# mzbac/mlx_sharding

Measured on AMD Instinct MI355X. Metric: output tokens/sec (decode), deepseek-v2-lite PP, higher is better.
Workload: dtype bf16; 1 GPU; model=deepseek-v2-lite, global_batch=64, seq_len=512, parallelism=pp1, micro_batches=1, weights=int4-w4a16

## Files before the change

### mlx_sharding_amd/models/deepseek_v2.py

```python

from __future__ import annotations

from typing import Dict, List, Optional, Tuple

import torch
import torch.nn as nn

from .. import ops
from ..config import ModelConfig, QuantConfig, ShardSpec
from ..ops.kvcache import KVCache
from .base import Linear, RMSNorm, StageModel, owned_layer_indices
from .llama import LlamaMLP, _Inner


class SwitchMLP(nn.Module):

    def __init__(self, n_experts: int, hidden: int, inter: int,
                 quant: Optional[QuantConfig] = None,
                 dtype: torch.dtype = torch.bfloat16):
        super().__init__()
        self.n_experts = n_experts
        self.quant = quant
        self.gate_proj = _StackedLinear(n_experts, hidden, inter, quant, dtype)
        self.up_proj = _StackedLinear(n_experts, hidden, inter, quant, dtype)
        self.down_proj = _StackedLinear(n_experts, inter, hidden, quant, dtype)

    def resident_dense(self):
        if self.quant is None:
            return None
        g, u, d = self.gate_proj, self.up_proj, self.down_proj
        return ops.expert_dequant_resident(
            (g.weight, g.scales, g.biases),
            (u.weight, u.scales, u.biases),
            (d.weight, d.scales, d.biases),
            self.quant.group_size, self.quant.bits)

    def forward_subs(self, x_flat: torch.Tensor, subs,
                     max_tok: int = 4) -> torch.Tensor:
        if self.quant is not None:
            import os
            if os.environ.get("MLXS_AMD_MOE_RESIDENT"):
                dense = self.resident_dense()
                if dense is not None:
                    return ops.grouped_expert_mlp_subs(
                        x_flat, dense[0], dense[1], dense[2], subs, max_tok)
            g, u, d = self.gate_proj, self.up_proj, self.down_proj
            return ops.grouped_expert_mlp_quant_subs(
                x_flat,
                (g.weight, g.scales, g.biases),
                (u.weight, u.scales, u.biases),
                (d.weight, d.scales, d.biases),
                subs, self.quant.group_size, self.quant.bits)
        return ops.grouped_expert_mlp_subs(
            x_flat, self.gate_proj.weight, self.up_proj.weight,
            self.down_proj.weight, subs, max_tok)

    def forward(self, x_flat: torch.Tensor, weights: torch.Tensor,
                indices: torch.Tensor) -> torch.Tensor:
        if self.quant is not None:
            g, u, d = self.gate_proj, self.up_proj, self.down_proj
            return ops.grouped_expert_mlp_quant(
                x_flat,
                (g.weight, g.scales, g.biases),
                (u.weight, u.scales, u.biases),
                (d.weight, d.scales, d.biases),
                weights, indices, self.quant.group_size, self.quant.bits)
        return ops.grouped_expert_mlp(
            x_flat, self.gate_proj.weight, self.up_proj.weight,
            self.down_proj.weight, weights, indices)


class _StackedLinear(nn.Module):

    def __init__(self, E: int, in_features: int, out_features: int,
                 quant: Optional[QuantConfig], dtype: torch.dtype):
        super().__init__()
        self.quantc = quant
        if quant is None:
            self.weight = nn.Parameter(
                torch.empty(E, out_features, in_features, dtype=dtype),
                requires_grad=False)
        else:
            per_word = 32 // quant.bits
            wdtype = torch.uint32 if hasattr(torch, "uint32") else torch.int32
            self.weight = nn.Parameter(
                torch.empty(E, out_features, in_features // per_word, dtype=wdtype),
                requires_grad=False)
            self.scales = nn.Parameter(
                torch.empty(E, out_features, in_features // quant.group_size, dtype=dtype),
                requires_grad=False)
            self.biases = nn.Parameter(
                torch.empty(E, out_features, in_features // quant.group_size, dtype=dtype),
                requires_grad=False)

    def dense(self) -> torch.Tensor:
        if self.quantc is None:
            return self.weight
        outs = [ops.dequantize(self.weight[e], self.scales[e], self.biases[e],
                               self.quantc.group_size, self.quantc.bits)
                for e in range(self.weight.shape[0])]
        return torch.stack(outs)


class MLAAttention(nn.Module):
    def __init__(self, cfg: ModelConfig, quant_for, prefix: str):
        super().__init__()
        H = cfg.hidden_size
        self.n_heads = cfg["num_attention_heads"]
        self.qk_nope = int(cfg.get("qk_nope_head_dim", 128))
        self.qk_rope = int(cfg.get("qk_rope_head_dim", 64))
        self.v_head_dim = int(cfg.get("v_head_dim", 128))
        self.kv_lora_rank = int(cfg.get("kv_lora_rank", 512))
        self.q_lora_rank = cfg.get("q_lora_rank")
        self.qk_head_dim = self.qk_nope + self.qk_rope
        q = lambda name: quant_for(f"{prefix}.{name}")
        eps = cfg.get("rms_norm_eps", 1e-6)
        if self.q_lora_rank:
            self.q_a_proj = Linear(H, self.q_lora_rank, q("q_a_proj"))
            self.q_a_layernorm = RMSNorm(self.q_lora_rank, eps)
            self.q_b_proj = Linear(self.q_lora_rank, self.n_heads * self.qk_head_dim,
                                   q("q_b_proj"))
        else:
            self.q_proj = Linear(H, self.n_heads * self.qk_head_dim, q("q_proj"))
        self._fused_qkv = None
        self.kv_a_proj_with_mqa = Linear(H, self.kv_lora_rank + self.qk_rope,
                                         q("kv_a_proj_with_mqa"))
        self.kv_a_layernorm = RMSNorm(self.kv_lora_rank, eps)
        self.kv_b_proj = Linear(self.kv_lora_rank,
                                self.n_heads * (self.qk_nope + self.v_head_dim),
                                q("kv_b_proj"))
        self.o_proj = Linear(self.n_heads * self.v_head_dim, H, q("o_proj"))

        rs = cfg.get("rope_scaling") or {}
        mscale_all = float(rs.get("mscale_all_dim", 0.0) or 0.0)
        factor = float(rs.get("factor", 1.0))
        scale = self.qk_head_dim ** -0.5
        if mscale_all and factor > 1.0:
            scale = scale * ops.yarn_mscale(factor, mscale_all) ** 2
        self.scale = scale
        self._w_uk = None
        self._w_uv = None

    def absorbed_supported(self) -> bool:
        ext = ops.hip_ext()
        if ext is None:
            return False
        dk = self.kv_lora_rank + self.qk_rope
        return (dk % 8 == 0 and self.kv_lora_rank % 8 == 0
                and ext.attn_decode_shape_ok(self.n_heads, self.kv_lora_rank))

    def _ensure_absorb(self, device, dtype):
        if self._w_uk is not None:
            return
        w = self.kv_b_proj.weight
        if self.kv_b_proj.quant is not None:
            qc = self.kv_b_proj.quant
            w = ops.dequantize(w, self.kv_b_proj.scales, self.kv_b_proj.biases,
                               qc.group_size, qc.bits)
        w = w.to(device=device, dtype=dtype)
        w = w.view(self.n_heads, self.qk_nope + self.v_head_dim,
                   self.kv_lora_rank)
        self._w_uk = w[:, : self.qk_nope, :].contiguous()
        self._w_uv = w[:, self.qk_nope:, :].transpose(1, 2).contiguous()

    def forward(self, x, cos, sin, cache: Optional[KVCache]):
        if cache is not None and cache.n_kv_heads == 1 and self.n_heads > 1:
            return self._forward_absorbed(x, cos, sin, cache)
        return self._forward_naive(x, cos, sin, cache)

    def _forward_absorbed(self, x, cos, sin, cache: KVCache):
        B, T, _ = x.shape
        nh, rank, rope = self.n_heads, self.kv_lora_rank, self.qk_rope
        ckv = None
        if self._fused_qkv is not None:
            qh, ckv = self._fused_qkv(x)
        elif self.q_lora_rank:
            qh = self.q_b_proj(self.q_a_layernorm(self.q_a_proj(x)))
        else:
            qh = self.q_proj(x)
        qh = qh.view(B, T, nh, self.qk_head_dim)
        q_nope = qh[..., : self.qk_nope]
        q_pe = ops.apply_rope(qh[..., self.qk_nope:], cos, sin,
                              interleaved=True)

        if ckv is None:
            ckv = self.kv_a_proj_with_mqa(x)
        c_kv, k_pe = ckv.split([rank, rope], dim=-1)
        c_kv = self.kv_a_layernorm(c_kv)
        k_pe = ops.apply_rope(k_pe.view(B, T, 1, rope), cos, sin,
                              interleaved=True).view(B, T, rope)

        gp = cache.graph_pos
        offset = 0 if gp is not None else cache.offset
        if ops.use_native(x):
            k_all, _ = cache.append_mla(c_kv.reshape(B, T, 1, rank), k_pe)
        else:
            row = torch.cat([c_kv, k_pe], dim=-1).unsqueeze(1)
            k_all, _ = cache.update(row, row[..., :0])

        if T == 1:
            self._ensure_absorb(x.device, x.dtype)
            qn = q_nope.permute(2, 0, 1, 3).reshape(nh, B * T, self.qk_nope)
            q_abs = torch.bmm(qn, self._w_uk)
            qf = torch.cat([q_abs.view(nh, B, T, rank).permute(1, 0, 2, 3),
                            q_pe.transpose(1, 2)], dim=-1)
            o = ops.attention(qf, k_all, k_all[..., :rank], self.scale,
                              causal_offset=offset, pos_dev=gp)
            ov = torch.bmm(o.permute(1, 0, 2, 3).reshape(nh, B * T, rank),
                           self._w_uv)
            out = ov.view(nh, B, T, self.v_head_dim).permute(1, 2, 0, 3)
            return self.o_proj(out.reshape(B, T, -1))

        S = k_all.shape[2] if gp is not None else cache.offset
        ckv_all = k_all[:, 0, :S, :rank]
        kpe_all = k_all[:, 0, :S, rank:]
        kvh = self.kv_b_proj(ckv_all).view(B, S, nh,
                                           self.qk_nope + self.v_head_dim)
        ext = ops.hip_ext() if ops.use_native(x) else None
        if ext is not None:
            k = kvh.new_empty(B, nh, S, self.qk_head_dim)
            v = kvh.new_empty(B, nh, S, self.v_head_dim)
            ext.mla_append_kv(kvh, kpe_all, k, v, pos0=0)
        else:
            k = torch.cat([kvh[..., : self.qk_nope],
                           kpe_all.reshape(B, S, 1, rope)
                           .expand(B, S, nh, rope)],
                          dim=-1).transpose(1, 2).contiguous()
            v = kvh[..., self.qk_nope:].transpose(1, 2).contiguous()
        qf = torch.cat([q_nope, q_pe], dim=-1).transpose(1, 2)
        out = ops.attention(qf, k, v, self.scale, causal_offset=offset)
        return self.o_proj(out.transpose(1, 2).reshape(B, T, -1))

    def _forward_naive(self, x, cos, sin, cache: Optional[KVCache]):
        B, T, _ = x.shape
        ckv = None
        if self._fused_qkv is not None:
            qh, ckv = self._fused_qkv(x)
        elif self.q_lora_rank:
            qh = self.q_b_proj(self.q_a_layernorm(self.q_a_proj(x)))
        else:
            qh = self.q_proj(x)
        qh = qh.view(B, T, self.n_heads, self.qk_head_dim)
        q_nope = qh[..., : self.qk_nope]
        q_pe = qh[..., self.qk_nope:]

        if ckv is None:
            ckv = self.kv_a_proj_with_mqa(x)
        c_kv, k_pe = ckv.split([self.kv_lora_rank, self.qk_rope], dim=-1)
        c_kv = self.kv_a_layernorm(c_kv)
        kvh = self.kv_b_proj(c_kv).view(B, T, self.n_heads, self.qk_nope + self.v_head_dim)

        q_pe = ops.apply_rope(q_pe, cos, sin, interleaved=True)
        k_pe = ops.apply_rope(k_pe.view(B, T, 1, self.qk_rope), cos, sin,
                              interleaved=True)
        qf = torch.cat([q_nope, q_pe], dim=-1).transpose(1, 2)

        offset = 0
        gp = None
        if cache is not None and ops.use_native(x):
            gp = cache.graph_pos
            if gp is None:
                offset = cache.offset
            k, v = cache.append_mla(kvh, k_pe.reshape(B, T, self.qk_rope))
            if gp is None:
                pass
        else:
            k_nope = kvh[..., : self.qk_nope]
            v = kvh[..., self.qk_nope:].transpose(1, 2)
            k = torch.cat([k_nope,
                           k_pe.expand(B, T, self.n_heads, self.qk_rope)],
                          dim=-1).transpose(1, 2)
            if cache is not None:
                gp = cache.graph_pos
                if gp is None:
                    offset = cache.offset
                k, v = cache.update(k, v)
        out = ops.attention(qf, k, v, self.scale, causal_offset=offset,
                            pos_dev=gp)
        return self.o_proj(out.transpose(1, 2).reshape(B, T, -1))


class DeepseekV2MoE(nn.Module):
    def __init__(self, cfg: ModelConfig, quant_for, prefix: str):
        super().__init__()
        H = cfg.hidden_size
        I_moe = int(cfg.get("moe_intermediate_size", 1408))
        self.n_experts = int(cfg.get("n_routed_experts", 64))
        self.top_k = int(cfg.get("num_experts_per_tok", 6))
        self.n_group = int(cfg.get("n_group", 1) or 1)
        self.topk_group = int(cfg.get("topk_group", 1) or 1)
        self.topk_method = cfg.get("topk_method", "greedy")
        self.routed_scaling_factor = float(cfg.get("routed_scaling_factor", 1.0))
        self.norm_topk_prob = bool(cfg.get("norm_topk_prob", False))
        self.gate = Linear(H, self.n_experts, None, dtype=torch.bfloat16)
        squant = quant_for(f"{prefix}.switch_mlp.gate_proj")
        self.switch_mlp = SwitchMLP(self.n_experts, H, I_moe, squant)
        n_shared = int(cfg.get("n_shared_experts", 0) or 0)
        if n_shared:
            shared_cfg = ModelConfig(cfg.model_type, dict(cfg.raw))
            shared_cfg.raw["intermediate_size"] = I_moe * n_shared
            self.shared_experts = LlamaMLP(shared_cfg, quant_for,
                                           f"{prefix}.shared_experts")
        else:
            self.shared_experts = None

    def _gate_groups(self) -> Tuple[int, int]:
        if self.topk_method == "group_limited_greedy":
            return self.n_group, self.topk_group
        return 1, 1

    def _fused_gate_ok(self, n_tokens: int) -> bool:
        E, K = self.n_experts, self.top_k
        n_group, topk_group = self._gate_groups()
        return (n_tokens <= 128 and 1 <= E <= 256 and 1 <= K <= 8
                and 1 <= n_group <= 32 and E % n_group == 0
                and 1 <= topk_group <= n_group
                and topk_group * (E // n_group) >= K)

    def forward(self, x):
        B, T, H = x.shape
        flat = x.reshape(-1, H)
        if (ops.use_native(flat)
                and self._fused_gate_ok(flat.shape[0])):
            logits = self.gate(flat.to(self.gate.weight.dtype))
            mt = 16
            n_group, topk_group = self._gate_groups()
            subs = ops.moe_gate_subranges(logits, self.top_k,
                                          self.routed_scaling_factor,
                                          self.norm_topk_prob, max_tok=mt,
                                          n_group=n_group,
                                          topk_group=topk_group)
            y = self.switch_mlp.forward_subs(flat, subs, mt)
        else:
            logits = self.gate(flat.to(self.gate.weight.dtype)).float()
            n_group = self.n_group if self.topk_method == "group_limited_greedy" else 1
            w, idx = ops.moe_gate(logits, self.top_k, n_group, self.topk_group,
                                  self.routed_scaling_factor, self.norm_topk_prob)
            w = w.to(x.dtype)
            y = self.switch_mlp(flat, w, idx)
        if self.shared_experts is not None:
            y = y + self.shared_experts(flat)
        return y.reshape(B, T, H)


class DeepseekV2DecoderLayer(nn.Module):
    def __init__(self, cfg: ModelConfig, quant_for, prefix: str, layer_idx: int):
        super().__init__()
        eps = cfg.get("rms_norm_eps", 1e-6)
        self.self_attn = MLAAttention(cfg, quant_for, f"{prefix}.self_attn")
        first_dense = int(cfg.get("first_k_dense_replace", 0))
        freq = int(cfg.get("moe_layer_freq", 1))
        is_moe = (cfg.get("n_routed_experts") is not None
                  and layer_idx >= first_dense and layer_idx % freq == 0)
        if is_moe:
            self.mlp = DeepseekV2MoE(cfg, quant_for, f"{prefix}.mlp")
        else:
            self.mlp = LlamaMLP(cfg, quant_for, f"{prefix}.mlp")
        self.input_layernorm = RMSNorm(cfg.hidden_size, eps)
        self.post_attention_layernorm = RMSNorm(cfg.hidden_size, eps)

    def forward(self, x, cos, sin, cache):
        attn = self.self_attn(self.input_layernorm(x), cos, sin, cache)
        pn = self.post_attention_layernorm
        y, h = ops.rms_norm_residual(attn, x, pn.weight, pn.eps,
                                     pn.weight_offset)
        return h + self.mlp(y)


class DeepseekV2StageModel(StageModel):
    model_type = "deepseek_v2"

    def __init__(self, config: ModelConfig, shard: ShardSpec, quant_for=None):
        super().__init__(config, shard)
        quant_for = quant_for or (lambda prefix: None)
        H = config.hidden_size
        self.model = _Inner()
        if shard.is_first:
            self.model.embed_tokens = nn.Embedding(config.vocab_size, H,
                                                   dtype=torch.bfloat16)
        layers = nn.ModuleDict()
        for i in owned_layer_indices(shard):
            layers[str(i)] = DeepseekV2DecoderLayer(config, quant_for,
                                                    f"model.layers.{i}", i)
        self.model.layers = layers
        if shard.is_last:
            self.model.norm = RMSNorm(H, config.get("rms_norm_eps", 1e-6))
            self.lm_head = Linear(H, config.vocab_size, quant_for("lm_head"))
        inv = ops.rope_freqs(int(config.get("qk_rope_head_dim", 64)),
                             float(config.get("rope_theta", 10000.0)),
                             config.get("rope_scaling"))
        rs = config.get("rope_scaling") or {}
        factor = float(rs.get("factor", 1.0))
        mscale = float(rs.get("mscale", 1.0) or 1.0)
        mscale_all = float(rs.get("mscale_all_dim", 0.0) or 0.0)
        if rs:
            num = ops.yarn_mscale(factor, mscale)
            den = ops.yarn_mscale(factor, mscale_all) if mscale_all else 1.0
            self.rope_attn_scale = num / den
        else:
            self.rope_attn_scale = 1.0
        self.register_buffer("rope_inv_freq", inv, persistent=False)

    @classmethod
    def sanitize(cls, weights: Dict[str, torch.Tensor], shard: ShardSpec) -> Dict[str, torch.Tensor]:
        out = dict(weights)
        expert_groups: Dict[str, Dict[int, str]] = {}
        for k in list(out.keys()):
            parts = k.split(".")
            if "experts" in parts and "shared_experts" not in k:
                ei = parts.index("experts")
                e = int(parts[ei + 1])
                stacked_key = ".".join(parts[:ei]) + ".switch_mlp." + ".".join(parts[ei + 2:])
                expert_groups.setdefault(stacked_key, {})[e] = k
        for stacked_key, members in expert_groups.items():
            n = max(members) + 1
            out[stacked_key] = torch.stack([out.pop(members[e]) for e in range(n)])
        return StageModel.sanitize.__func__(cls, out, shard)

    def cache_specs(self) -> List[Tuple[int, int, int]]:
        cfg = self.config
        if self._use_absorbed():
            rank = int(cfg.get("kv_lora_rank", 512))
            rope = int(cfg.get("qk_rope_head_dim", 64))
            return [(1, rank + rope, 0) for _ in range(self.shard.n_layers)]
        qk = int(cfg.get("qk_nope_head_dim", 128)) + int(cfg.get("qk_rope_head_dim", 64))
        vd = int(cfg.get("v_head_dim", 128))
        nh = cfg["num_attention_heads"]
        return [(nh, qk, vd) for _ in range(self.shard.n_layers)]

    def _use_absorbed(self) -> bool:
        try:
            p = next(self.parameters())
        except StopIteration:
            return False
        if not p.is_cuda:
            return False
        for layer in self.model.layers.values():
            return layer.self_attn.absorbed_supported()
        return False

    def forward(self, x: torch.Tensor, cache: Optional[List[KVCache]] = None) -> torch.Tensor:
        h = self.model.embed_tokens(x) if self.shard.is_first else x
        T = h.shape[1]
        cos, sin, _ = self.rope_for(cache[0] if cache else None, T, h.device)
        for j, i in enumerate(owned_layer_indices(self.shard)):
            c = cache[j] if cache is not None else None
            h = self.model.layers[str(i)](h, cos, sin, c)
        if self.shard.is_last:
            h = self.model.norm(h)
            h = self.lm_head(h)
        return h
```

### mlx_sharding_amd/ops/__init__.py

```python

from __future__ import annotations

import os
from typing import Optional

import torch

from . import reference as ref

_EXT = None
_EXT_ERR: Optional[str] = None
_TRIED = False


def _load_ext():
    global _EXT, _EXT_ERR, _TRIED
    if _TRIED:
        return _EXT
    _TRIED = True
    try:
        from mlx_sharding_amd import _hip_ops
        _EXT = _hip_ops
    except Exception as e:
        _EXT = None
        _EXT_ERR = repr(e)
    return _EXT


def hip_ext():
    return _load_ext()


def _force_torch() -> bool:
    return os.environ.get("MLXS_AMD_FORCE_TORCH", "0") == "1"


def _require_ext(op_name: str):
    ext = _load_ext()
    if ext is None:
        raise RuntimeError(
            f"mlx_sharding_amd: op '{op_name}' called on a GPU tensor but the "
            f"HIP extension mlx_sharding_amd._hip_ops is not importable "
            f"({_EXT_ERR}). Build it with `python setup.py build_ext --inplace` "
            f"(or __graft_entry__.build()). Refusing to fall back to eager torch "
            f"on GPU; set MLXS_AMD_FORCE_TORCH=1 only for debugging."
        )
    return ext


def _use_hip(t: torch.Tensor) -> bool:
    return t.is_cuda and not _force_torch()


def use_native(t: torch.Tensor) -> bool:
    return t.is_cuda and not _force_torch() and _load_ext() is not None



def rms_norm(x, weight, eps: float = 1e-5, weight_offset: float = 0.0):
    if _use_hip(x):
        return _require_ext("rms_norm").rms_norm(x, weight, eps, weight_offset)
    return ref.rms_norm(x, weight, eps, weight_offset)


def rms_norm_residual(x, residual, weight, eps: float = 1e-5, weight_offset: float = 0.0):
    if _use_hip(x):
        y, h = _require_ext("rms_norm_residual").rms_norm_residual(
            x, residual, weight, eps, weight_offset)
        return y, h
    h = x + residual
    return ref.rms_norm(h, weight, eps, weight_offset), h


def apply_rope(x, cos, sin, interleaved: bool = False):
    if _use_hip(x):
        return _require_ext("apply_rope").apply_rope(
            x, cos.contiguous(), sin.contiguous(), interleaved)
    return ref.apply_rope(x, cos, sin, interleaved)


def attention(q, k, v, scale: float, causal_offset: int = 0,
              softcap: float = 0.0, sliding_window: int = 0, pos_dev=None):
    if _use_hip(q):
        ext = _require_ext("attention")
        cache_layout = k.stride(3) == 1 and k.stride(2) == k.shape[3]
        if q.shape[2] == 1 and cache_layout:
            return ext.attn_decode(q, k, v, scale, softcap, sliding_window,
                                   pos_dev)
        if (cache_layout
                and ext.attn_prefill_shape_ok(q.shape[3], v.shape[3])):
            return ext.attn_prefill(q, k, v, scale, softcap, sliding_window,
                                    causal_offset)
        return _prefill_attention_gpu(q, k, v, scale, causal_offset,
                                      softcap, sliding_window)
    if pos_dev is not None:
        if pos_dev.numel() > 1:
            outs = []
            for b, p in enumerate(pos_dev.tolist()):
                outs.append(ref.attention(
                    q[b:b + 1], k[b:b + 1, :, :p + 1], v[b:b + 1, :, :p + 1],
                    scale, causal_offset=p, softcap=softcap,
                    sliding_window=sliding_window))
            return torch.cat(outs, dim=0)
        S = int(pos_dev.item()) + 1
        return ref.attention(q, k[:, :, :S], v[:, :, :S], scale,
                             causal_offset=S - 1, softcap=softcap,
                             sliding_window=sliding_window)
    return ref.attention(q, k, v, scale, causal_offset, softcap, sliding_window)


def _prefill_attention_gpu(q, k, v, scale, causal_offset, softcap, sliding_window):
    B, Hq, Tq, Dk = q.shape
    Hkv, S = k.shape[1], k.shape[2]
    G = Hq // Hkv
    qg = q.view(B, Hkv, G, Tq, Dk)
    scores = torch.matmul(qg, k.unsqueeze(2).transpose(-1, -2)).float() * scale
    if softcap and softcap > 0:
        scores = torch.tanh(scores / softcap) * softcap
    qpos = torch.arange(Tq, device=q.device)[:, None] + causal_offset
    kpos = torch.arange(S, device=q.device)[None, :]
    mask = kpos > qpos
    if sliding_window and sliding_window > 0:
        mask = mask | (kpos <= qpos - sliding_window)
    scores = scores.masked_fill(mask, float("-inf"))
    probs = torch.softmax(scores, dim=-1).to(q.dtype)
    out = torch.matmul(probs, v.unsqueeze(2))
    return out.reshape(B, Hq, Tq, v.shape[3])


def swiglu(gate, up):
    if _use_hip(gate):
        return _require_ext("swiglu").glu(gate, up, False)
    return ref.swiglu(gate, up)


def geglu(gate, up):
    if _use_hip(gate):
        return _require_ext("geglu").glu(gate, up, True)
    return ref.geglu(gate, up)


def softcap(x, cap: float):
    if _use_hip(x):
        return _require_ext("softcap").softcap(x, cap)
    return ref.softcap(x, cap)


_GEMV_MAX_M = 64
_LONG_K = 16384


_DQ_CACHE_BYTES = 0


def _dq_cache_cap() -> Optional[float]:
    if os.environ.get("MLXS_AMD_NO_DQ_CACHE"):
        return None
    return float(os.environ.get("MLXS_AMD_DQ_CACHE_GB", "96")) * (1 << 30)


def _dq_cache_ok(nbytes: int) -> bool:
    global _DQ_CACHE_BYTES
    cap = _dq_cache_cap()
    if cap is None or _DQ_CACHE_BYTES + nbytes > cap:
        return False
    _DQ_CACHE_BYTES += nbytes
    return True


def _small_m_route(M: int, O: int, K: int, x_dtype, w_dtype,
                   w_contiguous: bool, on_gpu: bool):
    if not (on_gpu and x_dtype == torch.bfloat16
            and w_dtype == torch.bfloat16 and w_contiguous
            and 0 < M <= _GEMV_MAX_M):
        return None
    if os.environ.get("MLXS_AMD_DENSE_GEMV") and K % 32 == 0:
        return "gemv", None
    if os.environ.get("MLXS_AMD_GEMM64") and K >= _LONG_K and K % 8 == 0:
        return "gemm64", None
    if (not os.environ.get("MLXS_AMD_NO_KSEG")
            and K >= _LONG_K and O >= 8192 and K % 256 == 0):
        return "kseg", max(1, min(16, 512 // max(1, O // 64)))
    return None


def _small_m_linear(x, weight, bias, name: str, ksegs):
    ext = _require_ext("linear")
    x2 = x.reshape(-1, x.shape[-1])
    if name == "gemv":
        y = ext.dense_gemv(x2, weight)
    elif name == "gemm64":
        y = ext.dense_gemm64(x2, weight)
    else:
        y = ext.gemm_m64_kseg(x2, weight, ksegs)
    if bias is not None:
        y = y + bias
    return y.reshape(*x.shape[:-1], y.shape[-1])


def linear(x, weight, bias=None):
    K = weight.shape[-1]
    if K >= _LONG_K or os.environ.get("MLXS_AMD_DENSE_GEMV"):
        route = _small_m_route(x.numel() // max(1, x.shape[-1]),
                               weight.shape[0], K, x.dtype, weight.dtype,
                               weight.is_contiguous(), _use_hip(x))
        if route is not None:
            return _small_m_linear(x, weight, bias, *route)
    return torch.nn.functional.linear(x, weight, bias)


def quantized_linear(x, w_q, scales, biases, group_size: int, bits: int):
    if _use_hip(x):
        ext = _require_ext("quantized_linear")
        lead = x.shape[:-1]
        H = x.shape[-1]
        x2 = x.reshape(-1, H)
        M = x2.shape[0]
        w = getattr(w_q, "_mlxs_dqw", None)
        O = w_q.shape[0]
        if w is None and _dq_cache_ok(O * H * 2):
            w = ext.dequant(w_q, scales, biases, H, group_size, bits)
            w_q._mlxs_dqw = w
        if w is not None:
            y = linear(x2, w)
        elif (M <= _GEMV_MAX_M and group_size in (32, 64, 128)
              and not os.environ.get("MLXS_AMD_NO_W4F16")):
            y = ext.w4f16_gemv(_to_f16_cached(x).reshape(-1, H),
                               repack_w4(w_q, bits),
                               scales, biases, group_size, bits)
        elif M <= _GEMV_MAX_M:
            y = ext.w4a16_gemv(x2, w_q, scales, biases, group_size, bits)
        else:
            w = ext.dequant(w_q, scales, biases, H, group_size, bits)
            y = torch.nn.functional.linear(x2, w)
        return y.reshape(*lead, y.shape[-1])
    return ref.quantized_linear(x, w_q, scales, biases, group_size, bits)


def moe_gate(router_logits, top_k: int, n_group: int = 1, topk_group: int = 1,
             routed_scaling_factor: float = 1.0, norm_topk_prob: bool = False):
    return ref.moe_gate(router_logits, top_k, n_group, topk_group,
                        routed_scaling_factor, norm_topk_prob)


_MOE_GEMM_MIN_N = 256


def make_expert_subranges(indices: torch.Tensor, weights: torch.Tensor,
                          n_experts: int, max_tok: int = 4):
    N, K = indices.shape
    P = N * K
    dev = indices.device
    flat_e = indices.reshape(-1).long()
    order = torch.argsort(flat_e, stable=True)
    tok = torch.arange(N, device=dev, dtype=torch.int64).repeat_interleave(K)
    sorted_tok = tok[order].to(torch.int32)
    sorted_wt = weights.reshape(-1).float()[order].contiguous()
    counts = torch.bincount(flat_e, minlength=n_experts)
    start = torch.cumsum(counts, 0) - counts
    nsub = (counts + max_tok - 1) // max_tok
    sub_start = torch.cumsum(nsub, 0) - nsub
    s_upper = n_experts + P // max_tok
    marker = torch.full((s_upper + 1,), -1, dtype=torch.int64, device=dev)
    eidx_all = torch.arange(n_experts, device=dev)
    src = torch.where(nsub > 0, eidx_all, torch.full_like(eidx_all, -1))
    marker.scatter_reduce_(0, sub_start, src, reduce="amax",
                           include_self=True)
    sub_expert = torch.cummax(marker[:s_upper], 0).values.clamp(min=0)
    sub_idx = torch.arange(s_upper, device=dev) - sub_start[sub_expert]
    sub_off = (start[sub_expert] + max_tok * sub_idx).to(torch.int32)
    sub_cnt = (counts[sub_expert] - max_tok * sub_idx) \
        .clamp(0, max_tok).to(torch.int32)
    return (sub_expert.to(torch.int32).contiguous(), sub_off.contiguous(),
            sub_cnt.contiguous(), sorted_tok.contiguous(), sorted_wt, order)


def _cached_t(w: torch.Tensor) -> torch.Tensor:
    if w.requires_grad or not w.is_leaf:
        return w.transpose(1, 2).contiguous()
    t = getattr(w, "_mlxs_t", None)
    if t is None:
        t = w.transpose(1, 2).contiguous()
        w._mlxs_t = t
    return t


def _cached_gu_t(gate_w: torch.Tensor, up_w: torch.Tensor) -> torch.Tensor:
    t = getattr(gate_w, "_mlxs_gut", None)
    if t is not None:
        return t
    E, I, H = gate_w.shape
    t = torch.empty(E, H, 2 * I, dtype=gate_w.dtype, device=gate_w.device)
    t[..., :I] = gate_w.transpose(1, 2)
    t[..., I:] = up_w.transpose(1, 2)
    if not gate_w.requires_grad and gate_w.is_leaf:
        gate_w._mlxs_gut = t
    return t


def _moe_prefill_gemm(x, gate_w, up_w, down_w, weights, indices,
                      dequant_all=None):
    N, K = indices.shape
    H = x.shape[-1]
    dev = x.device
    flat_e = indices.reshape(-1).long()
    order = torch.argsort(flat_e, stable=True)
    sorted_e = flat_e[order]
    tok = torch.arange(N, device=dev).repeat_interleave(K)[order]
    wts = weights.reshape(-1).float()[order]
    if dequant_all is not None:
        gate_w, up_w, down_w = dequant_all()
    E = gate_w.shape[0]
    counts = torch.zeros(E, dtype=torch.long, device=dev)
    counts.scatter_add_(0, sorted_e, torch.ones_like(sorted_e))
    start = torch.cumsum(counts, 0) - counts
    cap = (int(counts.max()) + 127) // 128 * 128
    P = N * K
    slot = torch.arange(P, device=dev) - start[sorted_e]
    dst = sorted_e * cap + slot
    xp = x.new_zeros(E * cap, H)
    ext = hip_ext() if x.is_cuda else None
    if ext is not None and H % 4 == 0:
        ext.moe_scatter_rows(x, xp, tok.to(torch.int32),
                             dst.to(torch.int32))
    else:
        xp[dst] = x[tok]
    xp = xp.view(E, cap, H)
    I = gate_w.shape[1]
    gu = torch.bmm(xp, _cached_gu_t(gate_w, up_w))
    hh = swiglu(gu[..., :I], gu[..., I:])
    d = torch.bmm(hh, _cached_t(down_w)).reshape(E * cap, H)
    if ext is not None and H % 4 == 0:
        inv = torch.empty_like(order)
        inv[order] = torch.arange(P, device=dev)
        pair_pos = dst[inv].view(N, K).to(torch.int32)
        pair_wts = weights.reshape(N, K).float()
        return ext.moe_gather_reduce(d, pair_pos, pair_wts, N)
    y = d[dst].float() * wts[:, None]
    out = torch.zeros(N, H, device=dev, dtype=torch.float32)
    out.index_add_(0, tok, y)
    return out.to(x.dtype)


def moe_gate_subranges(router_logits_bf16, top_k: int,
                       routed_scaling_factor: float = 1.0,
                       norm_topk_prob: bool = False, max_tok: int = 4,
                       n_group: int = 1, topk_group: int = 1):
    ext = _require_ext("moe_gate_subranges")
    N, E = router_logits_bf16.shape
    s_upper = E + (N * top_k) // max_tok
    return tuple(ext.moe_gate_subranges(router_logits_bf16, top_k, s_upper,
                                        max_tok, routed_scaling_factor,
                                        norm_topk_prob, n_group, topk_group))


def grouped_expert_mlp_subs(x, gate_w, up_w, down_w, subs, max_tok: int = 4):
    ext = _require_ext("grouped_expert_mlp")
    sub_e, sub_off, sub_cnt, sorted_tok, sorted_wt = subs
    P = sorted_tok.shape[0]
    h = ext.moe_gateup_grouped(x, gate_w, up_w, sub_e, sub_off, sub_cnt,
                               sorted_tok, P, max_tok)
    out = ext.moe_down_grouped(h, down_w, sub_e, sub_off, sub_cnt,
                               sorted_tok, sorted_wt, x.shape[0], max_tok)
    return out.to(x.dtype)


def _to_f16_cached(x: torch.Tensor) -> torch.Tensor:
    c = getattr(x, "_mlxs_f16", None)
    if c is not None:
        return c
    c = x.to(torch.float16)
    try:
        x._mlxs_f16 = c
    except Exception:
        pass
    return c


def repack_w4(wq: torch.Tensor, bits: int) -> torch.Tensor:
    cached = getattr(wq, "_mlxs_rp", None)
    if cached is not None:
        return cached
    w = wq.view(torch.int32).to(torch.int64) & 0xFFFFFFFF
    if bits == 4:
        even = ((w & 0xF) | (((w >> 8) & 0xF) << 4)
                | (((w >> 16) & 0xF) << 8) | (((w >> 24) & 0xF) << 12))
        odd = (((w >> 4) & 0xF) | (((w >> 12) & 0xF) << 4)
               | (((w >> 20) & 0xF) << 8) | (((w >> 28) & 0xF) << 12))
        rp = even | (odd << 16)
    elif bits == 8:
        rp = ((w & 0xFF) | (((w >> 16) & 0xFF) << 8)
              | (((w >> 8) & 0xFF) << 16) | (((w >> 24) & 0xFF) << 24))
    else:
        raise ValueError(f"unsupported bits {bits}")
    rp = torch.where(rp >= 2 ** 31, rp - 2 ** 32, rp).to(torch.int32)
    rp = rp.view(wq.dtype).contiguous()
    if not wq.requires_grad and wq.is_leaf:
        wq._mlxs_rp = rp
    return rp


def grouped_expert_mlp_quant_subs(x, gate, up, down, subs,
                                  group_size: int, bits: int):
    ext = _require_ext("grouped_expert_mlp_quant")
    sub_e, sub_off, sub_cnt, sorted_tok, sorted_wt = subs
    P = sorted_tok.shape[0]
    if group_size % 32 != 0 or x.shape[1] % 32 != 0:
        raise ValueError(
            "quantized experts require group_size % 32 == 0 and hidden % 32 "
            f"== 0 (got gs={group_size}, H={x.shape[1]})")
    x16 = _to_f16_cached(x)
    gq = repack_w4(gate[0], bits)
    uq = repack_w4(up[0], bits)
    dq = repack_w4(down[0], bits)
    hh = ext.moe_w4f16_gateup(x16, gq, uq, gate[1], gate[2], up[1], up[2],
                              sub_e, sub_off, sub_cnt, sorted_tok, P,
                              group_size, bits)
    out = ext.moe_w4f16_down(hh, dq, down[1], down[2], sub_e, sub_off,
                             sub_cnt, sorted_tok, sorted_wt, x.shape[0],
                             group_size, bits)
    return out.to(x.dtype)


def grouped_expert_mlp(x, gate_w, up_w, down_w, weights, indices):
    if _use_hip(x):
        _require_ext("grouped_expert_mlp")
        if x.shape[0] * indices.shape[1] >= _MOE_GEMM_MIN_N:
            return _moe_prefill_gemm(x, gate_w, up_w, down_w, weights, indices)
        E = gate_w.shape[0]
        sub_e, sub_off, sub_cnt, sorted_tok, sorted_wt, _ = \
            make_expert_subranges(indices, weights, E, max_tok=4)
        return grouped_expert_mlp_subs(
            x, gate_w, up_w, down_w,
            (sub_e, sub_off, sub_cnt, sorted_tok, sorted_wt))
    return ref.grouped_expert_mlp(x, gate_w, up_w, down_w, weights, indices)


def expert_dequant(gate, up, down, group_size: int, bits: int):
    cached = getattr(gate[0], "_mlxs_dq", None)
    if cached is not None:
        return cached
    ext = _require_ext("expert_dequant")
    E = gate[0].shape[0]
    pw = 32 // bits
    H = gate[0].shape[-1] * pw
    I = down[0].shape[-1] * pw
    gw = ext.dequant(gate[0].reshape(-1, H // pw), gate[1].reshape(-1, H // group_size),
                     gate[2].reshape(-1, H // group_size), H, group_size, bits)
    uw = ext.dequant(up[0].reshape(-1, H // pw), up[1].reshape(-1, H // group_size),
                     up[2].reshape(-1, H // group_size), H, group_size, bits)
    dw = ext.dequant(down[0].reshape(-1, I // pw), down[1].reshape(-1, I // group_size),
                     down[2].reshape(-1, I // group_size), I, group_size, bits)
    res = (gw.view(E, -1, H), uw.view(E, -1, H), dw.view(E, -1, I))
    if _dq_cache_ok(sum(t.numel() * 2 for t in res)):
        gate[0]._mlxs_dq = res
    return res


def expert_dequant_resident(gate, up, down, group_size: int, bits: int):
    cached = getattr(gate[0], "_mlxs_dq", None)
    if cached is not None:
        return cached
    pw = 32 // bits
    est = 2 * pw * (gate[0].numel() + up[0].numel() + down[0].numel())
    cap = _dq_cache_cap()
    if cap is None or _DQ_CACHE_BYTES + est > cap:
        return None
    res = expert_dequant(gate, up, down, group_size, bits)
    return res if getattr(gate[0], "_mlxs_dq", None) is not None else None


def grouped_expert_mlp_quant(x, gate, up, down, weights, indices,
                             group_size: int, bits: int):
    if _use_hip(x):
        _require_ext("grouped_expert_mlp_quant")
        E = gate[0].shape[0]
        if indices.numel() >= _MOE_GEMM_MIN_N:
            return _moe_prefill_gemm(
                x, None, None, None, weights, indices,
                dequant_all=lambda: expert_dequant(gate, up, down,
                                                   group_size, bits))
        sub_e, sub_off, sub_cnt, sorted_tok, sorted_wt, _ = \
            make_expert_subranges(indices, weights, E, max_tok=16)
        return grouped_expert_mlp_quant_subs(
            x, gate, up, down,
            (sub_e, sub_off, sub_cnt, sorted_tok, sorted_wt),
            group_size, bits)
    E = gate[0].shape[0]
    gw = torch.stack([ref.dequantize(gate[0][e], gate[1][e], gate[2][e],
                                     group_size, bits) for e in range(E)])
    uw = torch.stack([ref.dequantize(up[0][e], up[1][e], up[2][e],
                                     group_size, bits) for e in range(E)])
    dw = torch.stack([ref.dequantize(down[0][e], down[1][e], down[2][e],
                                     group_size, bits) for e in range(E)])
    return ref.grouped_expert_mlp(x, gw, uw, dw, weights, indices)



def sample(logits, temperature: float = 0.0, top_p: float = 1.0, generator=None):
    return ref.sample(logits, temperature, top_p, generator)


apply_repetition_penalty = ref.apply_repetition_penalty
rope_freqs = ref.rope_freqs
rope_cos_sin = ref.rope_cos_sin
yarn_mscale = ref.yarn_mscale
dequantize = ref.dequantize
quantize = ref.quantize
```

### mlx_sharding_amd/ops/hip/attn_decode.hip

```cpp

#include "hip_common.h"

#define AD_BLOCK 256

template <int G, int DVT>
__global__ __launch_bounds__(AD_BLOCK) void attn_decode_kernel(
    const short* __restrict__ q,
    const short* __restrict__ kcache,
    const short* __restrict__ vcache,
    short* __restrict__ out,
    float* __restrict__ part_o,
    float* __restrict__ part_ml,
    const int* __restrict__ s_ptr,
    int s_bstride,
    int B, int Hq, int Hkv, int S, long Scap, int Dk, int Dv, long vstride,
    float scale, float softcap, int window) {
  const int b = blockIdx.x / Hkv;
  if (s_ptr) S = s_ptr[b * s_bstride] + 1;
  const int hk = blockIdx.x % Hkv;
  const int split = blockIdx.y;
  const int nsplit = gridDim.y;
  const int hg = blockIdx.z;
  const int Gtot = (Hq / Hkv);
  const int h0 = hk * Gtot + hg * G;
  const int tid = threadIdx.x;

  extern __shared__ __attribute__((aligned(16))) char smem_raw[];
  short* q_lds = reinterpret_cast<short*>(smem_raw);
  float* p_lds = reinterpret_cast<float*>(
      smem_raw + (((size_t)G * Dk * sizeof(short) + 15) & ~(size_t)15));
  float* red = p_lds + (size_t)G * AD_BLOCK;

  for (int i = tid; i < G * Dk; i += AD_BLOCK) {
    int g = i / Dk, d = i % Dk;
    q_lds[i] = q[((long)b * Hq + h0 + g) * Dk + d];
  }
  __syncthreads();

  float m[G], l[G], acc[G * DVT];
#pragma unroll
  for (int g = 0; g < G; ++g) { m[g] = -1e30f; l[g] = 0.0f; }
#pragma unroll
  for (int i = 0; i < G * DVT; ++i) acc[i] = 0.0f;

  const long kbase = ((long)b * Hkv + hk) * Scap;
  int lo = (window > 0 && S > window) ? (S - window) : 0;
  int hi = S;
  if (nsplit > 1) {
    const long spanc = s_ptr ? Scap : (long)S;
    const long per = ((spanc + nsplit - 1) / nsplit + AD_BLOCK - 1)
                     / AD_BLOCK * AD_BLOCK;
    lo = max((long)lo, per * split);
    hi = min((long)S, per * (split + 1));
  }

  for (int tile = lo; tile < hi; tile += AD_BLOCK) {
    const int s_idx = tile + tid;
    float sc[G];
#pragma unroll
    for (int g = 0; g < G; ++g) sc[g] = -1e30f;
    if (s_idx < hi) {
      const short* krow = kcache + (kbase + s_idx) * Dk;
      float dot[G];
#pragma unroll
      for (int g = 0; g < G; ++g) dot[g] = 0.0f;
      int d0 = 0;
      for (; d0 + 64 <= Dk; d0 += 64) {
        bf16x8_t kc[8];
#pragma unroll
        for (int c = 0; c < 8; ++c)
          kc[c] = *reinterpret_cast<const bf16x8_t*>(krow + d0 + c * 8);
#pragma unroll
        for (int c = 0; c < 8; ++c)
#pragma unroll
          for (int g = 0; g < G; ++g) {
            bf16x8_t qv = *reinterpret_cast<const bf16x8_t*>(
                q_lds + (size_t)g * Dk + d0 + c * 8);
#pragma unroll
            for (int j = 0; j < 4; ++j)
              dot[g] = dot2_bf16(bf16x2_t{kc[c][2 * j], kc[c][2 * j + 1]},
                                 bf16x2_t{qv[2 * j], qv[2 * j + 1]}, dot[g]);
          }
      }
      for (; d0 < Dk; d0 += 8) {
        bf16x8_t kv = *reinterpret_cast<const bf16x8_t*>(krow + d0);
#pragma unroll
        for (int g = 0; g < G; ++g) {
          bf16x8_t qv =
              *reinterpret_cast<const bf16x8_t*>(q_lds + (size_t)g * Dk + d0);
#pragma unroll
          for (int j = 0; j < 4; ++j)
            dot[g] = dot2_bf16(bf16x2_t{kv[2 * j], kv[2 * j + 1]},
                               bf16x2_t{qv[2 * j], qv[2 * j + 1]}, dot[g]);
        }
      }
#pragma unroll
      for (int g = 0; g < G; ++g) {
        float v = dot[g] * scale;
        if (softcap > 0.0f) v = softcap * tanhf(v / softcap);
        sc[g] = v;
      }
    }
    constexpr int NW = AD_BLOCK / WAVE;
    const int lane = tid & (WAVE - 1);
    const int wid = tid / WAVE;
    float alpha[G];
#pragma unroll
    for (int g = 0; g < G; ++g) p_lds[(size_t)g * AD_BLOCK + tid] = sc[g];
    __syncthreads();
    for (int g = wid; g < G; g += NW) {
      float tm = -1e30f;
#pragma unroll
      for (int i = 0; i < NW; ++i)
        tm = fmaxf(tm, p_lds[(size_t)g * AD_BLOCK + lane + i * WAVE]);
      tm = wave_max(tm);
      if (lane == 0) red[g] = tm;
    }
    __syncthreads();
#pragma unroll
    for (int g = 0; g < G; ++g) {
      const float mnew = fmaxf(m[g], red[g]);
      alpha[g] = __expf(m[g] - mnew);
      float p = (s_idx < hi && sc[g] > -1e29f) ? __expf(sc[g] - mnew) : 0.0f;
      p_lds[(size_t)g * AD_BLOCK + tid] = p;
      m[g] = mnew;
    }
    __syncthreads();
    for (int g = wid; g < G; g += NW) {
      float ts = 0.0f;
#pragma unroll
      for (int i = 0; i < NW; ++i)
        ts += p_lds[(size_t)g * AD_BLOCK + lane + i * WAVE];
      ts = wave_sum(ts);
      if (lane == 0) red[g] = ts;
    }
    __syncthreads();
#pragma unroll
    for (int g = 0; g < G; ++g) l[g] = l[g] * alpha[g] + red[g];
    const int ntile = min(AD_BLOCK, hi - tile);
    const bf16* vbase = ((const bf16*)vcache) + (kbase + tile) * vstride + tid;
    float o[G * DVT];
#pragma unroll
    for (int i = 0; i < G * DVT; ++i) o[i] = 0.0f;
    if (tid < Dv) {
      long vcol[DVT];
      float vmask[DVT];
#pragma unroll
      for (int u = 0; u < DVT; ++u) {
        const int dv = tid + u * AD_BLOCK;
        vcol[u] = (dv < Dv) ? dv - tid : 0;
        vmask[u] = (dv < Dv) ? 1.0f : 0.0f;
      }
      int t = 0;
      for (; t + 8 <= ntile; t += 8) {
        float vv8[8][DVT];
#pragma unroll
        for (int tt = 0; tt < 8; ++tt)
#pragma unroll
          for (int u = 0; u < DVT; ++u)
            vv8[tt][u] =
                vmask[u] * bf2f(vbase[(long)(t + tt) * vstride + vcol[u]]);
#pragma unroll
        for (int tt = 0; tt < 8; ++tt)
#pragma unroll
          for (int g = 0; g < G; ++g) {
            const float p = p_lds[(size_t)g * AD_BLOCK + t + tt];
#pragma unroll
            for (int u = 0; u < DVT; ++u) o[g * DVT + u] += p * vv8[tt][u];
          }
      }
      for (; t < ntile; ++t) {
#pragma unroll
        for (int u = 0; u < DVT; ++u) {
          const float vv = vmask[u] * bf2f(vbase[(long)t * vstride + vcol[u]]);
#pragma unroll
          for (int g = 0; g < G; ++g)
            o[g * DVT + u] += p_lds[(size_t)g * AD_BLOCK + t] * vv;
        }
      }
    }
#pragma unroll
    for (int g = 0; g < G; ++g)
#pragma unroll
      for (int u = 0; u < DVT; ++u)
        acc[g * DVT + u] = acc[g * DVT + u] * alpha[g] + o[g * DVT + u];
    __syncthreads();
  }

  if (nsplit == 1) {
#pragma unroll
    for (int g = 0; g < G; ++g)
#pragma unroll
      for (int u = 0; u < DVT; ++u) {
        const int dv = tid + u * AD_BLOCK;
        if (dv < Dv)
          ((bf16*)out)[((long)b * Hq + h0 + g) * Dv + dv] =
              f2bf(acc[g * DVT + u] / l[g]);
      }
    return;
  }
#pragma unroll
  for (int g = 0; g < G; ++g)
#pragma unroll
    for (int u = 0; u < DVT; ++u) {
      const int dv = tid + u * AD_BLOCK;
      if (dv < Dv) {
        const long base = (((long)b * Hq + h0 + g) * nsplit + split) * Dv;
        part_o[base + dv] = acc[g * DVT + u];
      }
    }
  if (tid == 0) {
#pragma unroll
    for (int g = 0; g < G; ++g) {
      const long base = (((long)b * Hq + h0 + g) * nsplit + split) * 2;
      part_ml[base + 0] = m[g];
      part_ml[base + 1] = l[g];
    }
  }
}

__global__ void attn_decode_combine_kernel(
    const float* __restrict__ part_o,
    const float* __restrict__ part_ml,
    short* __restrict__ out,
    int NS, int Dv) {
  const long bh = blockIdx.x;
  const int tid = threadIdx.x;
  float mstar = -1e30f;
  for (int s = 0; s < NS; ++s)
    mstar = fmaxf(mstar, part_ml[(bh * NS + s) * 2]);
  float lsum = 0.0f;
  for (int s = 0; s < NS; ++s) {
    const float ms = part_ml[(bh * NS + s) * 2];
    const float ls = part_ml[(bh * NS + s) * 2 + 1];
    lsum += ls * __expf(ms - mstar);
  }
  for (int d = tid; d < Dv; d += blockDim.x) {
    float o = 0.0f;
    for (int s = 0; s < NS; ++s) {
      const float ms = part_ml[(bh * NS + s) * 2];
      o += part_o[(bh * NS + s) * Dv + d] * __expf(ms - mstar);
    }
    ((bf16*)out)[bh * Dv + d] = f2bf(o / lsum);
  }
}

extern "C" void launch_attn_decode(const void* q, const void* k, const void* v,
                                   void* out, float* part_o, float* part_ml,
                                   int nsplit, const int* s_ptr,
                                   int s_bstride, int B, int Hq,
                                   int Hkv, int S, long Scap, int Dk, int Dv,
                                   long vstride, float scale, float softcap,
                                   int window, hipStream_t stream) {
  const int Gtot = Hq / Hkv;
  const int DVT = (Dv + AD_BLOCK - 1) / AD_BLOCK;
  const int G = (Gtot == 16 && DVT == 2) ? 8 : Gtot;
  const int NHG = Gtot / G;
  const int nred = (G > AD_BLOCK / WAVE) ? G : AD_BLOCK / WAVE;
  size_t smem = (((size_t)G * Dk * sizeof(short) + 15) & ~(size_t)15) +
                ((size_t)G * AD_BLOCK + nred) * sizeof(float);
  dim3 grid((unsigned)(B * Hkv), (unsigned)nsplit, (unsigned)NHG);
  dim3 block(AD_BLOCK);
#define AD_CASE(GG, VT)                                                      \
  case GG * 16 + VT:                                                         \
    attn_decode_kernel<GG, VT><<<grid, block, smem, stream>>>(               \
        (const short*)q, (const short*)k, (const short*)v, (short*)out,      \
        part_o, part_ml, s_ptr, s_bstride, B, Hq, Hkv, S, Scap, Dk, Dv,      \
        vstride, scale, softcap, window);                                    \
    break;
  switch (G * 16 + DVT) {
    AD_CASE(1, 1)
    AD_CASE(2, 1)
    AD_CASE(4, 1)
    AD_CASE(4, 2)
    AD_CASE(8, 2)
    AD_CASE(16, 2)
    AD_CASE(6, 1)
    AD_CASE(7, 1)
    AD_CASE(8, 1)
    AD_CASE(16, 1)
    default:
      break;
  }
#undef AD_CASE
  if (nsplit > 1) {
    attn_decode_combine_kernel<<<dim3((unsigned)(B * Hq)), dim3(128), 0,
                                 stream>>>(part_o, part_ml, (short*)out,
                                           nsplit, Dv);
  }
}

extern "C" bool attn_decode_supported_shape(int G, int Dv) {
  if (Dv > 512) return false;
  const int dvt = (Dv + AD_BLOCK - 1) / AD_BLOCK;
  if (dvt == 2) return G == 16 || G == 4;
  return G == 1 || G == 2 || G == 4 || G == 6 || G == 7 || G == 8 ||
         G == 16;
}
```

### mlx_sharding_amd/ops/hip/bindings.hip

```cpp

#include <torch/extension.h>
#include <c10/hip/HIPStream.h>

#include "hip_common.h"

extern "C" {
void launch_rms_norm(const void*, void*, const void*, long, int, float, float,
                     long, hipStream_t);
void launch_rms_norm_residual(const void*, const void*, void*, void*,
                              const void*, long, int, float, float,
                              hipStream_t);
void launch_glu(const void*, const void*, void*, long, bool, hipStream_t);
void launch_glu_strided(const void*, const void*, void*, long, int, long,
                        long, bool, hipStream_t);
void launch_softcap(const void*, void*, long, float, hipStream_t);
void launch_rope(const void*, void*, const float*, const float*, long, int,
                 int, int, bool, long, long, long, hipStream_t);
void launch_mla_append_kv(const void*, const void*, void*, void*, const int*,
                          int, int, int, int, int, int, int, int, long, long,
                          hipStream_t);
void launch_rope_append_kv(const void*, const void*, const float*,
                           const float*, void*, void*, const int*, int, int,
                           int, int, int, int, long, bool, long, long, long,
                           hipStream_t);
void launch_attn_decode(const void*, const void*, const void*, void*, float*,
                        float*, int, const int*, int, int, int, int, int,
                        long, int, int, long, float, float, int, hipStream_t);
bool attn_decode_supported_shape(int, int);
void launch_attn_prefill(const void*, const void*, const void*, void*, int,
                         int, int, int, int, long, long, int, int, float,
                         float, int, int, hipStream_t);
bool attn_prefill_supported(int, int);
void launch_mfma_probe(const void*, const void*, float*, hipStream_t);
void launch_w4a16_gemv(const void*, const void*, const void*, const void*,
                       void*, int, int, int, int, int, hipStream_t);
int w4a16_mfma_nsplit(int, int, int);
void launch_bf16_gemv_mfma(const void*, const void*, void*, float*, int, int,
                           int, int, hipStream_t);
int bf16_gemv_nsplit(int, int, int);
void launch_bf16_gemm_m64(const void*, const void*, void*, float*, int, int,
                          int, int, hipStream_t);
int bf16_gemm_m64_nsplit(int, int, int);
void launch_w4a16_mfma(const void*, const void*, const void*, const void*,
                       void*, float*, int, int, int, int, int, int,
                       hipStream_t);
void launch_dequant(const void*, const void*, const void*, void*, long, int,
                    int, int, hipStream_t);
void launch_moe_scatter_rows(const void*, void*, const int*, const int*, int,
                             int, hipStream_t);
void launch_moe_gather_reduce(const void*, const int*, const float*, void*,
                              int, int, int, hipStream_t);
void launch_moe_gateup_mfma(const void*, const void*, const void*, void*,
                            const int*, const int*, const int*, const int*,
                            int, int, int, hipStream_t);
void launch_moe_down_mfma(const void*, const void*, float*, const int*,
                          const int*, const int*, const int*, const float*,
                          int, int, int, hipStream_t);
void launch_moe_gateup_grouped(const void*, const void*, const void*, void*,
                               const int*, const int*, const int*, const int*,
                               int, int, int, hipStream_t);
void launch_moe_down_grouped(const void*, const void*, float*, const int*,
                             const int*, const int*, const int*, const float*,
                             int, int, int, hipStream_t);
void launch_moe_w4_mfma(const void*, const void*, const void*, const void*,
                        void*, const int*, const int*, const int*,
                        const int*, int, int, int, int, int, hipStream_t);
void launch_moe_gate_subranges(const void*, int*, float*, int*, int*, int*,
                               int, int, int, int, int, float, int, int, int,
                               hipStream_t);
void launch_moe_w4f16_gateup(const void*, const void*, const void*,
                             const void*, const void*, const void*,
                             const void*, void*, const int*, const int*,
                             const int*, const int*, int, int, int, int, int,
                             hipStream_t);
void launch_moe_w4f16_down(const void*, const void*, const void*, const void*,
                           float*, const int*, const int*, const int*,
                           const int*, const float*, int, int, int, int, int,
                           hipStream_t);
void launch_w4f16_gemv(const void*, const void*, const void*, const void*,
                       void*, float*, int, int, int, int, int, int,
                       hipStream_t);
int w4f16_gemv_nsplit(int, int, int);
void launch_gemm_kseg(const void*, const void*, void*, void*, int, int, int,
                      int, hipStream_t);
void launch_gemm_kseg_w4(const void*, const void*, const void*, const void*,
                         void*, void*, int, int, int, int, int, hipStream_t);
}

namespace {

hipStream_t cur_stream() {
  return c10::hip::getCurrentHIPStream().stream();
}

void check_bf16(const torch::Tensor& t, const char* name) {
  TORCH_CHECK(t.is_cuda(), name, " must be on GPU");
  TORCH_CHECK(t.scalar_type() == torch::kBFloat16, name, " must be bf16");
}

bool row_view2(const torch::Tensor& t, long& rows, long& rstride) {
  const int d = t.dim();
  if (d < 2 || t.stride(d - 1) != 1) return false;
  if (d == 2) {
    rows = t.size(0);
    rstride = t.stride(0);
    return true;
  }
  if (d == 3) {
    if (t.stride(0) != t.size(1) * t.stride(1)) return false;
    rows = t.size(0) * t.size(1);
    rstride = t.stride(1);
    return true;
  }
  return false;
}

torch::Tensor splitk_scratch(int nk, int M, int O,
                             const torch::TensorOptions& opts) {
  if (nk <= 1) return torch::Tensor();
  return torch::empty({M, O}, opts.dtype(torch::kFloat32));
}

const int* pos_arg(const c10::optional<torch::Tensor>& pos, int B,
                   int& bstride) {
  bstride = 0;
  if (!pos.has_value()) return nullptr;
  TORCH_CHECK(pos->is_cuda() && pos->scalar_type() == torch::kInt32 &&
                  pos->is_contiguous(),
              "pos must be a contiguous int32 GPU tensor");
  const long n = pos->numel();
  TORCH_CHECK(n == 1 || n == B, "pos must hold 1 or B=", B,
              " positions, got ", n);
  bstride = (n == 1) ? 0 : 1;
  return pos->data_ptr<int>();
}

long rope_table_bstride(const torch::Tensor& cc, const torch::Tensor& sc,
                        int B, int T, int half) {
  TORCH_CHECK(cc.scalar_type() == torch::kFloat32 &&
                  sc.scalar_type() == torch::kFloat32, "cos/sin must be fp32");
  TORCH_CHECK(sc.sizes() == cc.sizes(), "cos/sin shape mismatch");
  if (cc.dim() == 3) {
    TORCH_CHECK(cc.size(0) == B && cc.size(1) == T && cc.size(2) == half,
                "cos shape mismatch: want [B, T, D/2]");
    return (long)T * half;
  }
  TORCH_CHECK(cc.dim() == 2 && cc.size(0) == T && cc.size(1) == half,
              "cos shape mismatch: want [T, D/2]");
  return 0;
}

float* f32_or_null(const torch::Tensor& t) {
  return t.defined() ? t.data_ptr<float>() : nullptr;
}

torch::Tensor rms_norm(torch::Tensor x, torch::Tensor w, double eps,
                       double w_off) {
  check_bf16(x, "x");
  check_bf16(w, "w");
  const int H = x.size(-1);
  TORCH_CHECK(H % 4 == 0, "H must be divisible by 4");
  long rows, rstride;
  torch::Tensor xv = x;
  if (!row_view2(x, rows, rstride) || rstride % 4 != 0
      || ((uintptr_t)x.data_ptr()) % 8 != 0) {
    xv = x.contiguous();
    rows = xv.numel() / H;
    rstride = H;
  }
  auto y = torch::empty(x.sizes(), x.options());
  launch_rms_norm(xv.data_ptr(), y.data_ptr(), w.contiguous().data_ptr(), rows,
                  H, (float)eps, (float)w_off, rstride, cur_stream());
  return y;
}

std::vector<torch::Tensor> rms_norm_residual(torch::Tensor x,
                                             torch::Tensor resid,
                                             torch::Tensor w, double eps,
                                             double w_off) {
  check_bf16(x, "x");
  auto xc = x.contiguous();
  auto rc = resid.contiguous();
  const int H = xc.size(-1);
  long rows = xc.numel() / H;
  auto y = torch::empty_like(xc);
  auto h = torch::empty_like(xc);
  launch_rms_norm_residual(xc.data_ptr(), rc.data_ptr(), y.data_ptr(),
                           h.data_ptr(), w.contiguous().data_ptr(), rows, H,
                           (float)eps, (float)w_off, cur_stream());
  return {y, h};
}

torch::Tensor glu(torch::Tensor gate, torch::Tensor up, bool gelu) {
  check_bf16(gate, "gate");
  TORCH_CHECK(gate.numel() == up.numel(), "gate/up size mismatch");
  TORCH_CHECK(gate.numel() % 4 == 0, "numel must be divisible by 4");
  const int I = gate.size(-1);
  long growz, gstride, urows, ustride;
  if (!(gate.is_contiguous() && up.is_contiguous())
      && row_view2(gate, growz, gstride) && row_view2(up, urows, ustride)
      && growz == urows && up.size(-1) == I && I % 4 == 0
      && gstride % 4 == 0 && ustride % 4 == 0
      && ((uintptr_t)gate.data_ptr()) % 8 == 0
      && ((uintptr_t)up.data_ptr()) % 8 == 0) {
    auto y = torch::empty(gate.sizes(), gate.options());
    launch_glu_strided(gate.data_ptr(), up.data_ptr(), y.data_ptr(), growz, I,
                       gstride, ustride, gelu, cur_stream());
    return y;
  }
  auto g = gate.contiguous();
  auto u = up.contiguous();
  auto y = torch::empty_like(g);
  launch_glu(g.data_ptr(), u.data_ptr(), y.data_ptr(), g.numel(), gelu,
             cur_stream());
  return y;
}

torch::Tensor softcap_op(torch::Tensor x, double cap) {
  check_bf16(x, "x");
  auto xc = x.contiguous();
  TORCH_CHECK(xc.numel() % 4 == 0, "numel must be divisible by 4");
  auto y = torch::empty_like(xc);
  launch_softcap(xc.data_ptr(), y.data_ptr(), xc.numel(), (float)cap,
                 cur_stream());
  return y;
}

torch::Tensor apply_rope(torch::Tensor x, torch::Tensor cos, torch::Tensor sin,
                         bool interleaved) {
  check_bf16(x, "x");
  TORCH_CHECK(x.dim() == 4, "x must be [B, T, nH, D]");
  auto cc = cos.contiguous();
  auto sc = sin.contiguous();
  const int B = x.size(0), T = x.size(1), nH = x.size(2), D = x.size(3);
  const long csb = rope_table_bstride(cc, sc, B, T, D / 2);
  torch::Tensor xv = x;
  long rstride = (long)nH * D, hstride = D;
  const bool strided_ok = x.stride(3) == 1
      && x.stride(0) == x.size(1) * x.stride(1);
  if (strided_ok) {
    rstride = x.stride(1);
    hstride = x.stride(2);
  } else {
    xv = x.contiguous();
  }
  auto y = torch::empty({B, T, nH, D}, x.options());
  launch_rope(xv.data_ptr(), y.data_ptr(), cc.data_ptr<float>(),
              sc.data_ptr<float>(), (long)B * T, T, nH, D, interleaved,
              rstride, hstride, csb, cur_stream());
  return y;
}

void rope_append_kv(torch::Tensor k, torch::Tensor v, torch::Tensor cos,
                    torch::Tensor sin, torch::Tensor kcache,
                    torch::Tensor vcache, c10::optional<torch::Tensor> pos,
                    int64_t pos0, bool interleaved) {
  check_bf16(k, "k");
  TORCH_CHECK(k.dim() == 4, "k must be [B, T, Hkv, D]");
  auto cc = cos.contiguous();
  auto sc = sin.contiguous();
  const int B = k.size(0), T = k.size(1), Hkv = k.size(2), D = k.size(3);
  TORCH_CHECK(D % 2 == 0, "head dim must be even");
  const long csb = rope_table_bstride(cc, sc, B, T, D / 2);
  TORCH_CHECK(kcache.is_contiguous() && vcache.is_contiguous(),
              "caches contiguous");
  TORCH_CHECK(kcache.size(3) == D && vcache.size(3) == D, "cache D mismatch");
  const long Scap = kcache.size(2);
  int pbs;
  const int* pp = pos_arg(pos, B, pbs);
  auto view_ok = [&](const torch::Tensor& t) {
    return t.stride(3) == 1 && t.stride(2) == D
        && t.stride(0) == t.size(1) * t.stride(1);
  };
  torch::Tensor kv = k, vv = v;
  long krs = (long)Hkv * D, vrs = (long)Hkv * D;
  if (view_ok(k)) krs = k.stride(1); else kv = k.contiguous();
  if (view_ok(v)) vrs = v.stride(1); else vv = v.contiguous();
  launch_rope_append_kv(kv.data_ptr(), vv.data_ptr(), cc.data_ptr<float>(),
                        sc.data_ptr<float>(), kcache.data_ptr(),
                        vcache.data_ptr(), pp, pbs, (int)pos0, B, T, Hkv, D,
                        Scap, interleaved, krs, vrs, csb, cur_stream());
}

void mla_append_kv(torch::Tensor kvh, torch::Tensor kpe, torch::Tensor kcache,
                   torch::Tensor vcache, c10::optional<torch::Tensor> pos,
                   int64_t pos0) {
  check_bf16(kvh, "kvh");
  const int B = kvh.size(0), T = kvh.size(1), nh = kvh.size(2);
  const int rope = kpe.size(-1);
  const int kd = kcache.size(3);
  const int vd = vcache.size(3);
  const int nope = kd - rope;
  TORCH_CHECK(kvh.size(3) == nope + vd, "kvh dim mismatch");
  TORCH_CHECK(kcache.is_contiguous() && vcache.is_contiguous(), "caches contiguous");
  const long Scap = kcache.size(2);
  int pbs;
  const int* pp = pos_arg(pos, B, pbs);
  long kpe_rows, kpe_rs;
  torch::Tensor kpev = kpe;
  if (!row_view2(kpe, kpe_rows, kpe_rs)) {
    kpev = kpe.contiguous();
    kpe_rs = rope;
  }
  launch_mla_append_kv(kvh.contiguous().data_ptr(), kpev.data_ptr(),
                       kcache.data_ptr(), vcache.data_ptr(), pp, pbs,
                       (int)pos0, B, T, nh, nope, vd, rope, Scap, kpe_rs,
                       cur_stream());
}

torch::Tensor attn_decode(torch::Tensor q, torch::Tensor k, torch::Tensor v,
                          double scale, double softcap, int64_t window,
                          c10::optional<torch::Tensor> pos) {
  check_bf16(q, "q");
  check_bf16(k, "k");
  TORCH_CHECK(q.size(2) == 1, "attn_decode needs Tq == 1");
  auto qc = q.contiguous();
  const int B = qc.size(0), Hq = qc.size(1), Dk = qc.size(3);
  const int Hkv = k.size(1), S = k.size(2);
  const int Dv = v.size(3);
  TORCH_CHECK(k.stride(3) == 1 && v.stride(3) == 1, "K/V rows must be contiguous");
  TORCH_CHECK(k.stride(2) == Dk, "K seq stride mismatch");
  const long vstride = v.stride(2);
  TORCH_CHECK(vstride >= Dv, "V seq stride too small");
  TORCH_CHECK(Hq % Hkv == 0, "Hq must be divisible by Hkv");
  TORCH_CHECK(Dk % 8 == 0, "Dk must be a multiple of 8");
  TORCH_CHECK(attn_decode_supported_shape(Hq / Hkv, Dv),
              "unsupported GQA ratio/Dv ", Hq / Hkv, " ", Dv);
  TORCH_CHECK(Dv <= 512, "Dv too large");
  long kScap = k.stride(1) / Dk;
  long vScap = v.stride(1) / vstride;
  TORCH_CHECK(kScap == vScap, "K/V capacity mismatch");
  auto out = torch::empty({B, Hq, 1, Dv}, qc.options());
  int sbs;
  const int* s_ptr = pos_arg(pos, B, sbs);
  long span = s_ptr ? kScap : (long)S;
  long slice = (B * Hkv <= 64) ? 256 : 512;
  int nsplit = (int)std::min<long>(
      std::min<long>(8, std::max<long>(1, 1024 / std::max(1, B * Hkv))),
      std::max<long>(1, (span + slice - 1) / slice));
  float* part_o = nullptr;
  float* part_ml = nullptr;
  torch::Tensor po, pml;
  if (nsplit > 1) {
    auto fopts = qc.options().dtype(torch::kFloat32);
    po = torch::empty({(long)B * Hq * nsplit * Dv}, fopts);
    pml = torch::empty({(long)B * Hq * nsplit * 2}, fopts);
    part_o = po.data_ptr<float>();
    part_ml = pml.data_ptr<float>();
  }
  launch_attn_decode(qc.data_ptr(), k.data_ptr(), v.data_ptr(),
                     out.data_ptr(), part_o, part_ml, nsplit, s_ptr, sbs, B,
                     Hq, Hkv, S, kScap, Dk, Dv, vstride, (float)scale,
                     (float)softcap, (int)window, cur_stream());
  return out;
}

torch::Tensor attn_prefill(torch::Tensor q, torch::Tensor k, torch::Tensor v,
                           double scale, double softcap, int64_t window,
                           int64_t causal_offset) {
  check_bf16(q, "q");
  auto qc = q.contiguous();
  const int B = qc.size(0), Hq = qc.size(1), T = qc.size(2), Dk = qc.size(3);
  const int Hkv = k.size(1), S = k.size(2), Dv = v.size(3);
  TORCH_CHECK(k.stride(3) == 1 && v.stride(3) == 1, "K/V rows must be contiguous");
  TORCH_CHECK(k.stride(2) == Dk && v.stride(2) == Dv, "K/V seq stride mismatch");
  TORCH_CHECK(Hq % Hkv == 0 && Dk % 32 == 0 && Dv % 16 == 0, "shape unsupported");
  TORCH_CHECK(Dk <= 256 && Dv <= 256, "Dk<=256, Dv<=256");
  TORCH_CHECK(attn_prefill_supported(Dk, Dv),
              "attn_prefill: no kernel instantiation for Dk=", Dk,
              " Dv=", Dv);
  long kScap = k.stride(1) / Dk;
  long vScap = v.stride(1) / Dv;
  auto out = torch::empty({B, Hq, T, Dv}, qc.options());
  launch_attn_prefill(qc.data_ptr(), k.data_ptr(), v.data_ptr(),
                      out.data_ptr(), B, Hq, Hkv, T, S, kScap, vScap, Dk, Dv,
                      (float)scale, (float)softcap, (int)window,
                      (int)causal_offset, cur_stream());
  return out;
}

torch::Tensor mfma_probe(torch::Tensor A, torch::Tensor Bm) {
  check_bf16(A, "A");
  auto D = torch::empty({16, 16}, A.options().dtype(torch::kFloat32));
  launch_mfma_probe(A.contiguous().data_ptr(), Bm.contiguous().data_ptr(),
                    D.data_ptr<float>(), cur_stream());
  return D;
}

torch::Tensor dense_gemv(torch::Tensor x, torch::Tensor w) {
  check_bf16(x, "x");
  check_bf16(w, "w");
  auto xc = x.contiguous();
  const int M = xc.size(0), H = xc.size(1);
  const int O = w.size(0);
  TORCH_CHECK(w.is_contiguous(), "w must be contiguous");
  TORCH_CHECK(M <= 64 && H % 32 == 0, "dense_gemv needs M<=64, H%32==0");
  auto y = torch::empty({M, O}, xc.options());
  const int nk = bf16_gemv_nsplit(M, O, H);
  auto yf = splitk_scratch(nk, M, O, xc.options());
  launch_bf16_gemv_mfma(xc.data_ptr(), w.data_ptr(), y.data_ptr(),
                        f32_or_null(yf), nk, M, O, H, cur_stream());
  return y;
}

torch::Tensor gemm_m64_kseg(torch::Tensor x, torch::Tensor w,
                            int64_t ksegs) {
  check_bf16(x, "x");
  check_bf16(w, "w");
  auto xc = x.contiguous();
  const int M = xc.size(0), K = xc.size(1);
  const int N = w.size(0);
  TORCH_CHECK(w.is_contiguous(), "w must be contiguous");
  TORCH_CHECK(M >= 1 && M <= 64 && K % 256 == 0,
              "gemm_m64_kseg needs 1<=M<=64, K%256==0");
  TORCH_CHECK(ksegs >= 1);
  auto yf = torch::empty({64, N}, xc.options().dtype(torch::kFloat32));
  auto y = torch::empty({M, N}, xc.options());
  launch_gemm_kseg(xc.data_ptr(), w.data_ptr(), yf.data_ptr<float>(),
                   y.data_ptr(), M, N, K, (int)ksegs, cur_stream());
  return y;
}

torch::Tensor gemm_m64_kseg_w4(torch::Tensor x, torch::Tensor wq,
                               torch::Tensor sc, torch::Tensor bi,
                               int64_t gs, int64_t ksegs) {
  TORCH_CHECK(x.scalar_type() == torch::kHalf, "x must be fp16");
  auto xc = x.contiguous();
  const int M = xc.size(0), K = xc.size(1);
  const int N = wq.size(0);
  TORCH_CHECK(wq.is_contiguous() && sc.is_contiguous() && bi.is_contiguous());
  TORCH_CHECK(M >= 1 && M <= 64 && K % 256 == 0,
              "gemm_m64_kseg_w4 needs 1<=M<=64, K%256==0");
  TORCH_CHECK(gs == 32 || gs == 64 || gs == 128, "gs must be 32/64/128");
  TORCH_CHECK(wq.size(1) == K / 8, "wq must be repacked w4 [N, K/8]");
  auto yf = torch::empty({64, N}, xc.options().dtype(torch::kFloat32));
  auto y = torch::empty({M, N}, xc.options().dtype(torch::kBFloat16));
  launch_gemm_kseg_w4(xc.data_ptr(), wq.data_ptr(), sc.data_ptr(),
                      bi.data_ptr(), yf.data_ptr<float>(), y.data_ptr(), M, N,
                      K, (int)gs, (int)ksegs, cur_stream());
  return y;
}

torch::Tensor dense_gemm64(torch::Tensor x, torch::Tensor w) {
  check_bf16(x, "x");
  check_bf16(w, "w");
  auto xc = x.contiguous();
  const int M = xc.size(0), H = xc.size(1);
  const int O = w.size(0);
  TORCH_CHECK(w.is_contiguous(), "w must be contiguous");
  TORCH_CHECK(M <= 64 && H % 8 == 0, "dense_gemm64 needs M<=64, H%8==0");
  auto y = torch::empty({M, O}, xc.options());
  const int nk = bf16_gemm_m64_nsplit(M, O, H);
  auto yf = splitk_scratch(nk, M, O, xc.options());
  launch_bf16_gemm_m64(xc.data_ptr(), w.data_ptr(), y.data_ptr(),
                       f32_or_null(yf), nk, M, O, H, cur_stream());
  return y;
}

torch::Tensor w4a16_gemv(torch::Tensor x, torch::Tensor wq,
                         torch::Tensor scales, torch::Tensor biases,
                         int64_t gs, int64_t bits) {
  check_bf16(x, "x");
  auto xc = x.contiguous();
  const int M = xc.size(0), H = xc.size(1);
  const int O = wq.size(0);
  auto y = torch::empty({M, O}, xc.options());
  if (M >= 8 && H % 32 == 0 && gs % 32 == 0) {
    const int nk = w4a16_mfma_nsplit(M, O, H);
    auto yf = splitk_scratch(nk, M, O, xc.options());
    launch_w4a16_mfma(xc.data_ptr(), wq.contiguous().data_ptr(),
                      scales.contiguous().data_ptr(),
                      biases.contiguous().data_ptr(), y.data_ptr(),
                      f32_or_null(yf), nk, M, O, H, (int)gs, (int)bits,
                      cur_stream());
  } else {
    launch_w4a16_gemv(xc.data_ptr(), wq.contiguous().data_ptr(),
                      scales.contiguous().data_ptr(),
                      biases.contiguous().data_ptr(), y.data_ptr(), M, O, H,
                      (int)gs, (int)bits, cur_stream());
  }
  return y;
}

torch::Tensor dequant(torch::Tensor wq, torch::Tensor scales,
                      torch::Tensor biases, int64_t H, int64_t gs,
                      int64_t bits) {
  const long O = wq.size(0);
  auto out = torch::empty({O, H}, scales.options());
  launch_dequant(wq.contiguous().data_ptr(), scales.contiguous().data_ptr(),
                 biases.contiguous().data_ptr(), out.data_ptr(), O, (int)H,
                 (int)gs, (int)bits, cur_stream());
  return out;
}

torch::Tensor moe_gateup_grouped(torch::Tensor x, torch::Tensor gate_w,
                                 torch::Tensor up_w, torch::Tensor sub_expert,
                                 torch::Tensor sub_off, torch::Tensor sub_cnt,
                                 torch::Tensor sorted_tok, int64_t P,
                                 int64_t max_tok) {
  check_bf16(x, "x");
  const int H = x.size(1);
  const int I = gate_w.size(1);
  const int S = sub_expert.size(0);
  TORCH_CHECK(sub_expert.scalar_type() == torch::kInt32, "sub arrays int32");
  auto h = torch::empty({P, I}, x.options());
  if (max_tok == 16 && H % 32 == 0 && I % 16 == 0) {
    launch_moe_gateup_mfma(
        x.contiguous().data_ptr(), gate_w.data_ptr(), up_w.data_ptr(),
        h.data_ptr(), sub_expert.data_ptr<int>(), sub_off.data_ptr<int>(),
        sub_cnt.data_ptr<int>(), sorted_tok.data_ptr<int>(), S, H, I,
        cur_stream());
  } else {
    TORCH_CHECK(max_tok <= 4, "scalar grouped kernel needs max_tok <= 4");
    TORCH_CHECK(H % 8 == 0 && I % 8 == 0,
                "scalar grouped kernel needs H % 8 == 0 and I % 8 == 0 (got H=",
                H, ", I=", I, ")");
    launch_moe_gateup_grouped(
        x.contiguous().data_ptr(), gate_w.data_ptr(), up_w.data_ptr(),
        h.data_ptr(), sub_expert.data_ptr<int>(), sub_off.data_ptr<int>(),
        sub_cnt.data_ptr<int>(), sorted_tok.data_ptr<int>(), S, H, I,
        cur_stream());
  }
  return h;
}

torch::Tensor moe_down_grouped(torch::Tensor h, torch::Tensor down_w,
                               torch::Tensor sub_expert, torch::Tensor sub_off,
                               torch::Tensor sub_cnt, torch::Tensor sorted_tok,
                               torch::Tensor sorted_wt, int64_t N,
                               int64_t max_tok) {
  const int I = h.size(1);
  const int H = down_w.size(1);
  const int S = sub_expert.size(0);
  auto out = torch::zeros({N, H}, h.options().dtype(torch::kFloat32));
  if (max_tok == 16 && I % 32 == 0 && H % 16 == 0) {
    launch_moe_down_mfma(
        h.contiguous().data_ptr(), down_w.data_ptr(), out.data_ptr<float>(),
        sub_expert.data_ptr<int>(), sub_off.data_ptr<int>(),
        sub_cnt.data_ptr<int>(), sorted_tok.data_ptr<int>(),
        sorted_wt.data_ptr<float>(), S, I, H, cur_stream());
  } else {
    TORCH_CHECK(max_tok <= 4, "scalar grouped kernel needs max_tok <= 4");
    TORCH_CHECK(H % 8 == 0 && I % 8 == 0,
                "scalar grouped kernel needs H % 8 == 0 and I % 8 == 0 (got H=",
                H, ", I=", I, ")");
    launch_moe_down_grouped(
        h.contiguous().data_ptr(), down_w.data_ptr(), out.data_ptr<float>(),
        sub_expert.data_ptr<int>(), sub_off.data_ptr<int>(),
        sub_cnt.data_ptr<int>(), sorted_tok.data_ptr<int>(),
        sorted_wt.data_ptr<float>(), S, I, H, cur_stream());
  }
  return out;
}

torch::Tensor moe_w4_mfma(torch::Tensor x, torch::Tensor wq,
                          torch::Tensor scales, torch::Tensor biases,
                          torch::Tensor sub_expert, torch::Tensor sub_off,
                          torch::Tensor sub_cnt, torch::Tensor sorted_tok,
                          int64_t P, int64_t gs, int64_t bits) {
  check_bf16(x, "x");
  const int H = x.size(1);
  const int O = wq.size(1);
  const int S = sub_expert.size(0);
  TORCH_CHECK(H % 32 == 0 && gs % 32 == 0, "H%32, gs%32 required");
  TORCH_CHECK(H % gs == 0, "moe_w4_mfma needs H % gs == 0 (got H=", H,
              ", gs=", gs, ")");
  auto y = torch::empty({P, O}, x.options());
  launch_moe_w4_mfma(x.contiguous().data_ptr(), wq.data_ptr(),
                     scales.data_ptr(), biases.data_ptr(), y.data_ptr(),
                     sub_expert.data_ptr<int>(), sub_off.data_ptr<int>(),
                     sub_cnt.data_ptr<int>(), sorted_tok.data_ptr<int>(), S,
                     H, O, (int)gs, (int)bits, cur_stream());
  return y;
}

torch::Tensor moe_w4f16_gateup(torch::Tensor x, torch::Tensor gq,
                               torch::Tensor uq, torch::Tensor gsc,
                               torch::Tensor gbi, torch::Tensor usc,
                               torch::Tensor ubi, torch::Tensor sub_expert,
                               torch::Tensor sub_off, torch::Tensor sub_cnt,
                               torch::Tensor sorted_tok, int64_t P,
                               int64_t gs, int64_t bits) {
  TORCH_CHECK(x.scalar_type() == torch::kHalf, "x must be fp16");
  const int H = x.size(1);
  const int I = gq.size(1);
  const int S = sub_expert.size(0);
  TORCH_CHECK(H % 32 == 0, "H%32 required");
  TORCH_CHECK(gs == 32 || gs == 64 || gs == 128, "gs must be 32/64/128");
  auto h = torch::empty({P, I}, x.options());
  launch_moe_w4f16_gateup(
      x.contiguous().data_ptr(), gq.data_ptr(), uq.data_ptr(), gsc.data_ptr(),
      gbi.data_ptr(), usc.data_ptr(), ubi.data_ptr(), h.data_ptr(),
      sub_expert.data_ptr<int>(), sub_off.data_ptr<int>(),
      sub_cnt.data_ptr<int>(), sorted_tok.data_ptr<int>(), S, H, I, (int)gs,
      (int)bits, cur_stream());
  return h;
}

torch::Tensor moe_w4f16_down(torch::Tensor hh, torch::Tensor dq,
                             torch::Tensor dsc, torch::Tensor dbi,
                             torch::Tensor sub_expert, torch::Tensor sub_off,
                             torch::Tensor sub_cnt, torch::Tensor sorted_tok,
                             torch::Tensor sorted_wt, int64_t N, int64_t gs,
                             int64_t bits) {
  TORCH_CHECK(hh.scalar_type() == torch::kHalf, "h must be fp16");
  const int I = hh.size(1);
  const int H = dq.size(1);
  const int S = sub_expert.size(0);
  TORCH_CHECK(I % 32 == 0, "I%32 required");
  TORCH_CHECK(gs == 32 || gs == 64 || gs == 128, "gs must be 32/64/128");
  auto out = torch::zeros({N, H}, hh.options().dtype(torch::kFloat32));
  launch_moe_w4f16_down(
      hh.contiguous().data_ptr(), dq.data_ptr(), dsc.data_ptr(),
      dbi.data_ptr(), out.data_ptr<float>(), sub_expert.data_ptr<int>(),
      sub_off.data_ptr<int>(), sub_cnt.data_ptr<int>(),
      sorted_tok.data_ptr<int>(), sorted_wt.data_ptr<float>(), S, I, H,
      (int)gs, (int)bits, cur_stream());
  return out;
}

torch::Tensor w4f16_gemv(torch::Tensor x, torch::Tensor wq,
                         torch::Tensor scales, torch::Tensor biases,
                         int64_t gs, int64_t bits) {
  TORCH_CHECK(x.scalar_type() == torch::kHalf, "x must be fp16");
  auto xc = x.contiguous();
  const int M = xc.size(0), H = xc.size(1);
  const int O = wq.size(0);
  TORCH_CHECK(M <= 64 && H % 32 == 0, "w4f16_gemv needs M<=64, H%32==0");
  TORCH_CHECK(gs == 32 || gs == 64 || gs == 128, "gs must be 32/64/128");
  auto y = torch::empty({M, O},
                        xc.options().dtype(torch::kBFloat16));
  const int nk = w4f16_gemv_nsplit(M, O, H);
  auto yf = splitk_scratch(nk, M, O, xc.options());
  launch_w4f16_gemv(xc.data_ptr(), wq.contiguous().data_ptr(),
                    scales.contiguous().data_ptr(),
                    biases.contiguous().data_ptr(), y.data_ptr(),
                    f32_or_null(yf), nk, M, O, H, (int)gs, (int)bits,
                    cur_stream());
  return y;
}

std::vector<torch::Tensor> moe_gate_subranges(torch::Tensor logits, int64_t K,
                                              int64_t s_upper, int64_t max_tok,
                                              double routed_scaling,
                                              bool norm_topk, int64_t n_group,
                                              int64_t topk_group) {
  check_bf16(logits, "logits");
  TORCH_CHECK(logits.dim() == 2, "logits must be [N, E]");
  auto lc = logits.contiguous();
  const int64_t N = lc.size(0), E = lc.size(1);
  TORCH_CHECK(N <= 128 && E >= 1 && E <= 256 && K >= 1 && K <= 8,
              "fused gate limits: N<=128, 1<=E<=256, 1<=K<=8 (got N=", N,
              ", E=", E, ", K=", K, ")");
  TORCH_CHECK(n_group >= 1 && n_group <= 32 && E % n_group == 0,
              "fused gate limits: 1<=n_group<=32 and E % n_group == 0 (got E=",
              E, ", n_group=", n_group, ")");
  TORCH_CHECK(topk_group >= 1 && topk_group <= n_group,
              "fused gate limits: 1<=topk_group<=n_group (got topk_group=",
              topk_group, ", n_group=", n_group, ")");
  TORCH_CHECK(topk_group * (E / n_group) >= K,
              "fused gate limits: topk_group*(E/n_group) >= K (got ",
              topk_group, "*", E / n_group, " < ", K, ")");
  TORCH_CHECK(max_tok >= 1 && s_upper >= E + (N * K) / max_tok,
              "fused gate needs max_tok>=1 and s_upper >= E + N*K/max_tok");
  const long P = (long)N * K;
  auto opts = torch::TensorOptions().dtype(torch::kInt32).device(lc.device());
  auto sorted_tok = torch::empty({P}, opts);
  auto sorted_wt = torch::empty({P}, opts.dtype(torch::kFloat32));
  auto sub_expert = torch::empty({s_upper}, opts);
  auto sub_off = torch::empty({s_upper}, opts);
  auto sub_cnt = torch::empty({s_upper}, opts);
  launch_moe_gate_subranges(lc.data_ptr(), sorted_tok.data_ptr<int>(),
                            sorted_wt.data_ptr<float>(),
                            sub_expert.data_ptr<int>(), sub_off.data_ptr<int>(),
                            sub_cnt.data_ptr<int>(), (int)N, (int)E, (int)K,
                            (int)s_upper, (int)max_tok, (float)routed_scaling,
                            norm_topk ? 1 : 0, (int)n_group, (int)topk_group,
                            cur_stream());
  return {sub_expert, sub_off, sub_cnt, sorted_tok, sorted_wt};
}

}

PYBIND11_MODULE(TORCH_EXTENSION_NAME, m) {
  m.def("rms_norm", &rms_norm, "fused RMSNorm (gfx950)");
  m.def("rms_norm_residual", &rms_norm_residual);
  m.def("glu", &glu);
  m.def("softcap", &softcap_op);
  m.def("apply_rope", &apply_rope);
  m.def("rope_append_kv", &rope_append_kv, pybind11::arg("k"),
        pybind11::arg("v"), pybind11::arg("cos"), pybind11::arg("sin"),
        pybind11::arg("kcache"), pybind11::arg("vcache"),
        pybind11::arg("pos") = pybind11::none(), pybind11::arg("pos0") = 0,
        pybind11::arg("interleaved") = false);
  m.def("mla_append_kv", &mla_append_kv,
        pybind11::arg("kvh"), pybind11::arg("kpe"), pybind11::arg("kcache"),
        pybind11::arg("vcache"), pybind11::arg("pos") = pybind11::none(),
        pybind11::arg("pos0") = 0);
  m.def("attn_decode", &attn_decode, pybind11::arg("q"), pybind11::arg("k"),
        pybind11::arg("v"), pybind11::arg("scale"), pybind11::arg("softcap"),
        pybind11::arg("window"), pybind11::arg("pos") = pybind11::none());
  m.def("attn_decode_shape_ok", [](int64_t g, int64_t dv) {
    return attn_decode_supported_shape((int)g, (int)dv);
  });
  m.def("attn_prefill", &attn_prefill);
  m.def("attn_prefill_shape_ok", [](int64_t dk, int64_t dv) {
    return attn_prefill_supported((int)dk, (int)dv);
  });
  m.def("mfma_probe", &mfma_probe);
  m.def("w4a16_gemv", &w4a16_gemv);
  m.def("w4f16_gemv", &w4f16_gemv);
  m.def("w4a16_mfma_nsplit", [](int64_t M, int64_t O, int64_t H) {
    return w4a16_mfma_nsplit((int)M, (int)O, (int)H);
  });
  m.def("w4f16_gemv_nsplit", [](int64_t M, int64_t O, int64_t H) {
    return w4f16_gemv_nsplit((int)M, (int)O, (int)H);
  });
  m.def("dense_gemv", &dense_gemv);
  m.def("dense_gemm64", &dense_gemm64);
  m.def("gemm_m64_kseg", &gemm_m64_kseg);
  m.def("gemm_m64_kseg_w4", &gemm_m64_kseg_w4);
  m.def("dequant", &dequant);
  m.def("moe_gateup_grouped", &moe_gateup_grouped);
  m.def("moe_down_grouped", &moe_down_grouped);
  m.def("moe_w4_mfma", &moe_w4_mfma);
  m.def("moe_w4f16_gateup", &moe_w4f16_gateup);
  m.def("moe_w4f16_down", &moe_w4f16_down);
  m.def("moe_gate_subranges", &moe_gate_subranges, pybind11::arg("logits"),
        pybind11::arg("top_k"), pybind11::arg("s_upper"),
        pybind11::arg("max_tok"), pybind11::arg("routed_scaling"),
        pybind11::arg("norm_topk"), pybind11::arg("n_group") = 1,
        pybind11::arg("topk_group") = 1);
  m.def("moe_scatter_rows",
        [](torch::Tensor src, torch::Tensor dst, torch::Tensor src_idx,
           torch::Tensor dst_idx) {
          check_bf16(src, "src");
          const int P = src_idx.size(0), H = src.size(-1);
          TORCH_CHECK(H % 4 == 0 && dst.size(-1) == H, "row shape");
          TORCH_CHECK(src_idx.scalar_type() == torch::kInt32 &&
                          dst_idx.scalar_type() == torch::kInt32,
                      "indices int32");
          launch_moe_scatter_rows(src.contiguous().data_ptr(), dst.data_ptr(),
                                  src_idx.data_ptr<int>(),
                                  dst_idx.data_ptr<int>(), P, H,
                                  cur_stream());
        });
  m.def("moe_gather_reduce",
        [](torch::Tensor d, torch::Tensor pos, torch::Tensor wts, int64_t N) {
          check_bf16(d, "d");
          const int K = pos.size(1), H = d.size(-1);
          TORCH_CHECK(pos.scalar_type() == torch::kInt32, "pos int32");
          TORCH_CHECK(wts.scalar_type() == torch::kFloat32, "wts fp32");
          auto out = torch::empty({N, H}, d.options());
          launch_moe_gather_reduce(d.contiguous().data_ptr(),
                                   pos.contiguous().data_ptr<int>(),
                                   wts.contiguous().data_ptr<float>(),
                                   out.data_ptr(), (int)N, K, H,
                                   cur_stream());
          return out;
        });
}
```

### mlx_sharding_amd/ops/hip/elementwise.hip

```cpp
#include "hip_common.h"


template <int BLOCK, bool RESIDUAL>
__global__ void rms_norm_kernel(const short* __restrict__ x,
                                const short* __restrict__ resid,
                                short* __restrict__ y,
                                short* __restrict__ h_out,
                                const short* __restrict__ w, int H, float eps,
                                float w_off, long xstride) {
  __shared__ float scratch[BLOCK / WAVE];
  const long row = blockIdx.x;
  const short* xr = x + row * xstride;
  const short* rr = RESIDUAL ? resid + row * H : nullptr;
  short* yr = y + row * H;
  short* hr = RESIDUAL ? h_out + row * H : nullptr;

  float ss = 0.0f;
  const int nvec = H / 4;
  const short4v* xv = reinterpret_cast<const short4v*>(xr);
  const short4v* rv = reinterpret_cast<const short4v*>(rr);
  for (int i = threadIdx.x; i < nvec; i += BLOCK) {
    short4v v = xv[i];
    float f0 = bfbits2f(v.x), f1 = bfbits2f(v.y), f2 = bfbits2f(v.z),
          f3 = bfbits2f(v.w);
    if (RESIDUAL) {
      short4v u = rv[i];
      f0 += bfbits2f(u.x); f1 += bfbits2f(u.y);
      f2 += bfbits2f(u.z); f3 += bfbits2f(u.w);
      short4v hv;
      hv.x = (short)__bfloat16_as_ushort(f2bf(f0));
      hv.y = (short)__bfloat16_as_ushort(f2bf(f1));
      hv.z = (short)__bfloat16_as_ushort(f2bf(f2));
      hv.w = (short)__bfloat16_as_ushort(f2bf(f3));
      reinterpret_cast<short4v*>(hr)[i] = hv;
      f0 = bfbits2f(hv.x); f1 = bfbits2f(hv.y);
      f2 = bfbits2f(hv.z); f3 = bfbits2f(hv.w);
    }
    ss += f0 * f0 + f1 * f1 + f2 * f2 + f3 * f3;
  }
  ss = block_sum<BLOCK>(ss, scratch);
  const float inv = rsqrtf(ss / (float)H + eps);

  const short4v* wv = reinterpret_cast<const short4v*>(w);
  const short4v* src = RESIDUAL ? reinterpret_cast<const short4v*>(hr)
                                : xv;
  for (int i = threadIdx.x; i < nvec; i += BLOCK) {
    short4v v = src[i];
    short4v wvv = wv[i];
    short4v o;
    o.x = (short)__bfloat16_as_ushort(f2bf(bfbits2f(v.x) * inv * (bfbits2f(wvv.x) + w_off)));
    o.y = (short)__bfloat16_as_ushort(f2bf(bfbits2f(v.y) * inv * (bfbits2f(wvv.y) + w_off)));
    o.z = (short)__bfloat16_as_ushort(f2bf(bfbits2f(v.z) * inv * (bfbits2f(wvv.z) + w_off)));
    o.w = (short)__bfloat16_as_ushort(f2bf(bfbits2f(v.w) * inv * (bfbits2f(wvv.w) + w_off)));
    reinterpret_cast<short4v*>(yr)[i] = o;
  }
}

extern "C" void launch_rms_norm(const void* x, void* y, const void* w,
                                long rows, int H, float eps, float w_off,
                                long xstride, hipStream_t stream) {
  constexpr int BLOCK = 256;
  rms_norm_kernel<BLOCK, false><<<dim3((unsigned)rows), dim3(BLOCK), 0, stream>>>(
      (const short*)x, nullptr, (short*)y, nullptr, (const short*)w, H, eps,
      w_off, xstride);
}

extern "C" void launch_rms_norm_residual(const void* x, const void* resid,
                                         void* y, void* h_out, const void* w,
                                         long rows, int H, float eps,
                                         float w_off, hipStream_t stream) {
  constexpr int BLOCK = 256;
  rms_norm_kernel<BLOCK, true><<<dim3((unsigned)rows), dim3(BLOCK), 0, stream>>>(
      (const short*)x, (const short*)resid, (short*)y, (short*)h_out,
      (const short*)w, H, eps, w_off, H);
}


template <bool GELU>
__global__ void glu_kernel(const short* __restrict__ gate,
                           const short* __restrict__ up,
                           short* __restrict__ y, long n4) {
  const long stride = (long)gridDim.x * blockDim.x;
  for (long i = blockIdx.x * blockDim.x + threadIdx.x; i < n4; i += stride) {
    short4v g = reinterpret_cast<const short4v*>(gate)[i];
    short4v u = reinterpret_cast<const short4v*>(up)[i];
    float gf[4] = {bfbits2f(g.x), bfbits2f(g.y), bfbits2f(g.z), bfbits2f(g.w)};
    float uf[4] = {bfbits2f(u.x), bfbits2f(u.y), bfbits2f(u.z), bfbits2f(u.w)};
    short4v o;
    short* op = reinterpret_cast<short*>(&o);
#pragma unroll
    for (int k = 0; k < 4; ++k) {
      float a;
      if (GELU) {
        float x = gf[k];
        float inner = 0.7978845608028654f * (x + 0.044715f * x * x * x);
        a = 0.5f * x * (1.0f + tanhf(inner));
      } else {
        a = gf[k] / (1.0f + __expf(-gf[k]));
      }
      op[k] = (short)__bfloat16_as_ushort(f2bf(a * uf[k]));
    }
    reinterpret_cast<short4v*>(y)[i] = o;
  }
}

template <bool GELU>
__global__ void glu_strided_kernel(const short* __restrict__ gate,
                                   const short* __restrict__ up,
                                   short* __restrict__ y, long rows, int I4,
                                   long gstride, long ustride) {
  const long total = rows * I4;
  const long stride = (long)gridDim.x * blockDim.x;
  for (long i = blockIdx.x * blockDim.x + threadIdx.x; i < total; i += stride) {
    const long r = i / I4;
    const int c = (int)(i - r * I4);
    short4v g = *reinterpret_cast<const short4v*>(gate + r * gstride + c * 4);
    short4v u = *reinterpret_cast<const short4v*>(up + r * ustride + c * 4);
    float gf[4] = {bfbits2f(g.x), bfbits2f(g.y), bfbits2f(g.z), bfbits2f(g.w)};
    float uf[4] = {bfbits2f(u.x), bfbits2f(u.y), bfbits2f(u.z), bfbits2f(u.w)};
    short4v o;
    short* op = reinterpret_cast<short*>(&o);
#pragma unroll
    for (int k = 0; k < 4; ++k) {
      float a;
      if (GELU) {
        float x = gf[k];
        float inner = 0.7978845608028654f * (x + 0.044715f * x * x * x);
        a = 0.5f * x * (1.0f + tanhf(inner));
      } else {
        a = gf[k] / (1.0f + __expf(-gf[k]));
      }
      op[k] = (short)__bfloat16_as_ushort(f2bf(a * uf[k]));
    }
    reinterpret_cast<short4v*>(y)[i] = o;
  }
}

extern "C" void launch_glu_strided(const void* gate, const void* up, void* y,
                                   long rows, int I, long gstride,
                                   long ustride, bool gelu,
                                   hipStream_t stream) {
  const long n4 = rows * (I / 4);
  int block = 256;
  long want = (n4 + block - 1) / block;
  int grid = (int)min(want, (long)(256 * 8));
  if (grid < 1) grid = 1;
  if (gelu)
    glu_strided_kernel<true><<<dim3(grid), dim3(block), 0, stream>>>(
        (const short*)gate, (const short*)up, (short*)y, rows, I / 4, gstride,
        ustride);
  else
    glu_strided_kernel<false><<<dim3(grid), dim3(block), 0, stream>>>(
        (const short*)gate, (const short*)up, (short*)y, rows, I / 4, gstride,
        ustride);
}

extern "C" void launch_glu(const void* gate, const void* up, void* y, long n,
                           bool gelu, hipStream_t stream) {
  long n4 = n / 4;
  int block = 256;
  long want = (n4 + block - 1) / block;
  int grid = (int)min(want, (long)(256 * 8));
  if (grid < 1) grid = 1;
  if (gelu)
    glu_kernel<true><<<dim3(grid), dim3(block), 0, stream>>>(
        (const short*)gate, (const short*)up, (short*)y, n4);
  else
    glu_kernel<false><<<dim3(grid), dim3(block), 0, stream>>>(
        (const short*)gate, (const short*)up, (short*)y, n4);
}


__global__ void softcap_kernel(const short* __restrict__ x, short* __restrict__ y,
                               long n4, float cap) {
  const long stride = (long)gridDim.x * blockDim.x;
  const float inv = 1.0f / cap;
  for (long i = blockIdx.x * blockDim.x + threadIdx.x; i < n4; i += stride) {
    short4v v = reinterpret_cast<const short4v*>(x)[i];
    short4v o;
    o.x = (short)__bfloat16_as_ushort(f2bf(cap * tanhf(bfbits2f(v.x) * inv)));
    o.y = (short)__bfloat16_as_ushort(f2bf(cap * tanhf(bfbits2f(v.y) * inv)));
    o.z = (short)__bfloat16_as_ushort(f2bf(cap * tanhf(bfbits2f(v.z) * inv)));
    o.w = (short)__bfloat16_as_ushort(f2bf(cap * tanhf(bfbits2f(v.w) * inv)));
    reinterpret_cast<short4v*>(y)[i] = o;
  }
}

extern "C" void launch_softcap(const void* x, void* y, long n, float cap,
                               hipStream_t stream) {
  long n4 = n / 4;
  int block = 256;
  long want = (n4 + block - 1) / block;
  int grid = (int)min(want, (long)(256 * 8));
  if (grid < 1) grid = 1;
  softcap_kernel<<<dim3(grid), dim3(block), 0, stream>>>(
      (const short*)x, (short*)y, n4, cap);
}


template <bool INTERLEAVED>
__global__ void rope_kernel(const short* __restrict__ x, short* __restrict__ y,
                            const float* __restrict__ cost,
                            const float* __restrict__ sint,
                            int T, int n_heads, int D, long xrstride,
                            int xhstride, long cs_bstride) {
  const int half = D / 2;
  const long bh = blockIdx.x;
  const long row = bh / n_heads;
  const int head = bh % n_heads;
  const int t = row % T;
  const short* xr = x + row * xrstride + (long)head * xhstride;
  short* yr = y + (row * n_heads + head) * D;
  const long cs_off = (row / T) * cs_bstride + (long)t * half;
  const float* c = cost + cs_off;
  const float* s = sint + cs_off;
  for (int p = threadIdx.x; p < half; p += blockDim.x) {
    float x1, x2;
    int i1, i2;
    if (INTERLEAVED) {
      i1 = 2 * p;
      i2 = 2 * p + 1;
    } else {
      i1 = p;
      i2 = p + half;
    }
    x1 = bfbits2f(xr[i1]);
    x2 = bfbits2f(xr[i2]);
    float o1 = x1 * c[p] - x2 * s[p];
    float o2 = x2 * c[p] + x1 * s[p];
    yr[i1] = (short)__bfloat16_as_ushort(f2bf(o1));
    yr[i2] = (short)__bfloat16_as_ushort(f2bf(o2));
  }
}

extern "C" void launch_rope(const void* x, void* y, const float* cost,
                            const float* sint, long rows, int T, int n_heads,
                            int D, bool interleaved, long xrstride,
                            long xhstride, long cs_bstride,
                            hipStream_t stream) {
  dim3 grid((unsigned)(rows * n_heads));
  int block = D / 2 < 64 ? 64 : (D / 2 > 256 ? 256 : D / 2);
  if (interleaved)
    rope_kernel<true><<<grid, dim3(block), 0, stream>>>(
        (const short*)x, (short*)y, cost, sint, T, n_heads, D, xrstride,
        (int)xhstride, cs_bstride);
  else
    rope_kernel<false><<<grid, dim3(block), 0, stream>>>(
        (const short*)x, (short*)y, cost, sint, T, n_heads, D, xrstride,
        (int)xhstride, cs_bstride);
}


__global__ void mla_append_kv_kernel(
    const short* __restrict__ kvh, const short* __restrict__ kpe,
    short* __restrict__ kcache, short* __restrict__ vcache,
    const int* __restrict__ pos_ptr, int pos_bstride, int pos0, int B, int T,
    int nh, int nope, int vd, int rope, long Scap, long kpe_rstride) {
  const int bh = blockIdx.x;
  const int t = blockIdx.y;
  const int b = bh / nh;
  const int h = bh % nh;
  const long pos = (pos_ptr ? pos_ptr[b * pos_bstride] : pos0) + t;
  const short* src = kvh + (((long)b * T + t) * nh + h) * (nope + vd);
  const short* pe = kpe + ((long)b * T + t) * kpe_rstride;
  short* krow = kcache + (((long)b * nh + h) * Scap + pos) * (nope + rope);
  short* vrow = vcache + (((long)b * nh + h) * Scap + pos) * vd;
  for (int i = threadIdx.x; i < nope; i += blockDim.x) krow[i] = src[i];
  for (int i = threadIdx.x; i < rope; i += blockDim.x) krow[nope + i] = pe[i];
  for (int i = threadIdx.x; i < vd; i += blockDim.x) vrow[i] = src[nope + i];
}


template <bool INTERLEAVED>
__global__ void rope_append_kv_kernel(
    const short* __restrict__ k, const short* __restrict__ v,
    const float* __restrict__ cost, const float* __restrict__ sint,
    short* __restrict__ kcache, short* __restrict__ vcache,
    const int* __restrict__ pos_ptr, int pos_bstride, int pos0, int B, int T,
    int Hkv, int D, long Scap, long k_rstride, long v_rstride,
    long cs_bstride) {
  const int bh = blockIdx.x;
  const int t = blockIdx.y;
  const int b = bh / Hkv;
  const int h = bh % Hkv;
  const long pos = (pos_ptr ? pos_ptr[b * pos_bstride] : pos0) + t;
  const short* kr = k + ((long)b * T + t) * k_rstride + (long)h * D;
  const short* vr = v + ((long)b * T + t) * v_rstride + (long)h * D;
  short* kd = kcache + (((long)b * Hkv + h) * Scap + pos) * D;
  short* vd = vcache + (((long)b * Hkv + h) * Scap + pos) * D;
  const int half = D / 2;
  const long cs_off = (long)b * cs_bstride + (long)t * half;
  const float* c = cost + cs_off;
  const float* s = sint + cs_off;
  for (int p = threadIdx.x; p < half; p += blockDim.x) {
    int i1, i2;
    if (INTERLEAVED) {
      i1 = 2 * p;
      i2 = 2 * p + 1;
    } else {
      i1 = p;
      i2 = p + half;
    }
    const float x1 = bfbits2f(kr[i1]), x2 = bfbits2f(kr[i2]);
    kd[i1] = (short)__bfloat16_as_ushort(f2bf(x1 * c[p] - x2 * s[p]));
    kd[i2] = (short)__bfloat16_as_ushort(f2bf(x2 * c[p] + x1 * s[p]));
    vd[i1] = vr[i1];
    vd[i2] = vr[i2];
  }
}

extern "C" void launch_rope_append_kv(const void* k, const void* v,
                                      const float* cost, const float* sint,
                                      void* kcache, void* vcache,
                                      const int* pos_ptr, int pos_bstride,
                                      int pos0, int B, int T, int Hkv, int D,
                                      long Scap, bool interleaved,
                                      long k_rstride, long v_rstride,
                                      long cs_bstride, hipStream_t stream) {
  dim3 grid((unsigned)(B * Hkv), (unsigned)T);
  int block = D / 2 < 64 ? 64 : (D / 2 > 256 ? 256 : D / 2);
  if (interleaved)
    rope_append_kv_kernel<true><<<grid, dim3(block), 0, stream>>>(
        (const short*)k, (const short*)v, cost, sint, (short*)kcache,
        (short*)vcache, pos_ptr, pos_bstride, pos0, B, T, Hkv, D, Scap,
        k_rstride, v_rstride, cs_bstride);
  else
    rope_append_kv_kernel<false><<<grid, dim3(block), 0, stream>>>(
        (const short*)k, (const short*)v, cost, sint, (short*)kcache,
        (short*)vcache, pos_ptr, pos_bstride, pos0, B, T, Hkv, D, Scap,
        k_rstride, v_rstride, cs_bstride);
}

extern "C" void launch_mla_append_kv(const void* kvh, const void* kpe,
                                     void* kcache, void* vcache,
                                     const int* pos_ptr, int pos_bstride,
                                     int pos0, int B, int T, int nh, int nope,
                                     int vd, int rope, long Scap,
                                     long kpe_rstride, hipStream_t stream) {
  mla_append_kv_kernel<<<dim3((unsigned)(B * nh), (unsigned)T), dim3(128), 0,
                         stream>>>((const short*)kvh, (const short*)kpe,
                                   (short*)kcache, (short*)vcache, pos_ptr,
                                   pos_bstride, pos0, B, T, nh, nope, vd,
                                   rope, Scap,
                                   kpe_rstride);
}
```

### mlx_sharding_amd/ops/hip/moe_w4f16.hip

```cpp

#include "hip_common.h"
#include "splitk.h"
#include "w4f16_dequant.h"

#define WF_WAVES 4
#define WF_BLOCK (WF_WAVES * WAVE)
#define WF_NSL 8

template <int GS>
struct LaneSB {
  static constexpr int NSEL = GS == 32 ? 2 : 1;
  f16x2 s2[NSEL], b2[NSEL];
  __device__ __forceinline__ void load(const short* srow, const short* brow,
                                       int sl, int q, float qoff) {
    int g0;
    if (GS == 32) g0 = sl + 2 * q;
    else if (GS == 64) g0 = sl / 2 + q;
    else g0 = sl / 4 + (q >= 2 ? 1 : 0);
#pragma unroll
    for (int c = 0; c < NSEL; ++c) {
      const float sf = bfbits2f(srow[g0 + c]);
      s2[c] = splat2(sf);
      b2[c] = splat2(bfbits2f(brow[g0 + c]) + qoff * sf);
    }
  }
  static __device__ __forceinline__ int sel(int i) {
    return GS == 32 ? i / 4 : 0;
  }
};

__device__ __forceinline__ int batch_kk(int sl, int q, int i) {
  return sl * 32 + q * 64 + i * 8;
}
static_assert(WF_NSL == 8, "batch_kk remap requires 8-slice batches");

template <int BITS, int GS>
__global__ __launch_bounds__(WF_BLOCK) void moe_w4f16_gateup_kernel(
    const _Float16* __restrict__ x, const unsigned int* __restrict__ gq,
    const unsigned int* __restrict__ uq, const short* __restrict__ gsc,
    const short* __restrict__ gbi, const short* __restrict__ usc,
    const short* __restrict__ ubi, _Float16* __restrict__ h,
    const int* __restrict__ sub_expert, const int* __restrict__ sub_off,
    const int* __restrict__ sub_cnt, const int* __restrict__ sorted_tok,
    int H, int I) {
  const int s = blockIdx.y;
  const int e = sub_expert[s];
  const int p0 = sub_off[s];
  const int cnt = sub_cnt[s];
  if (cnt == 0) return;
  const int lane = threadIdx.x & (WAVE - 1);
  const int wid = threadIdx.x / WAVE;
  const int wpr = H * BITS / 32;

  const int row0 = (blockIdx.x * WF_WAVES + wid) * 16;
  if (row0 >= I) return;
  const int wr = min(row0 + (lane & 15), I - 1);
  const long ebase = (long)e * I;
  const unsigned int* grow = gq + (ebase + wr) * wpr;
  const unsigned int* urow = uq + (ebase + wr) * wpr;
  const int ngr = H / GS;
  const short* gsr = gsc + (ebase + wr) * ngr;
  const short* gbr = gbi + (ebase + wr) * ngr;
  const short* usr = usc + (ebase + wr) * ngr;
  const short* ubr = ubi + (ebase + wr) * ngr;
  const _Float16* xrow =
      x + (long)sorted_tok[p0 + min(lane & 15, cnt - 1)] * H;

  float4v gacc = {0, 0, 0, 0}, uacc = {0, 0, 0, 0};
  float4v gacc2 = {0, 0, 0, 0}, uacc2 = {0, 0, 0, 0};
  constexpr float QOFF = BITS == 4 ? 8.0f : 128.0f;
  constexpr int WPS = BITS == 4 ? 1 : 2;

  const int nsl_total = H / 32;
  const int q = lane >> 4;
  int sl = 0;
  for (; sl + WF_NSL <= nsl_total; sl += WF_NSL) {
    uint4 gw4[2 * WPS], uw4[2 * WPS];
    const int w0 = batch_kk(sl, q, 0) * BITS / 32;
#pragma unroll
    for (int c = 0; c < 2 * WPS; ++c) {
      gw4[c] = *reinterpret_cast<const uint4*>(grow + w0 + c * 4);
      uw4[c] = *reinterpret_cast<const uint4*>(urow + w0 + c * 4);
    }
    f16x8 bv[WF_NSL];
#pragma unroll
    for (int i = 0; i < WF_NSL; ++i)
      bv[i] = *reinterpret_cast<const f16x8*>(xrow + batch_kk(sl, q, i));
    LaneSB<GS> gsb, usb;
    gsb.load(gsr, gbr, sl, q, QOFF);
    usb.load(usr, ubr, sl, q, QOFF);
    const unsigned int* gw = reinterpret_cast<const unsigned int*>(gw4);
    const unsigned int* uw = reinterpret_cast<const unsigned int*>(uw4);
    f16x8 ga[WF_NSL], ua[WF_NSL];
#pragma unroll
    for (int i = 0; i < WF_NSL; ++i) {
      const int c = LaneSB<GS>::sel(i);
      if (BITS == 4) {
        dq8<4>(gw[i], gsb.s2[c], gsb.b2[c], &ga[i]);
        dq8<4>(uw[i], usb.s2[c], usb.b2[c], &ua[i]);
      } else {
        dq8_w8(gw[i * 2], gw[i * 2 + 1], gsb.s2[c], gsb.b2[c], &ga[i]);
        dq8_w8(uw[i * 2], uw[i * 2 + 1], usb.s2[c], usb.b2[c], &ua[i]);
      }
    }
#pragma unroll
    for (int i = 0; i < WF_NSL; i += 2) {
      gacc = __builtin_amdgcn_mfma_f32_16x16x32_f16(ga[i], bv[i], gacc, 0, 0, 0);
      uacc = __builtin_amdgcn_mfma_f32_16x16x32_f16(ua[i], bv[i], uacc, 0, 0, 0);
      gacc2 = __builtin_amdgcn_mfma_f32_16x16x32_f16(ga[i + 1], bv[i + 1],
                                                     gacc2, 0, 0, 0);
      uacc2 = __builtin_amdgcn_mfma_f32_16x16x32_f16(ua[i + 1], bv[i + 1],
                                                     uacc2, 0, 0, 0);
    }
  }
  for (; sl < nsl_total; ++sl) {
    const int kk = sl * 32 + (lane >> 4) * 8;
    const float gsf = bfbits2f(gsr[kk / GS]);
    const float usf = bfbits2f(usr[kk / GS]);
    const f16x2 gs2 = splat2(gsf);
    const f16x2 gb2 = splat2(bfbits2f(gbr[kk / GS]) + QOFF * gsf);
    const f16x2 us2 = splat2(usf);
    const f16x2 ub2 = splat2(bfbits2f(ubr[kk / GS]) + QOFF * usf);
    f16x8 ga, ua;
    if (BITS == 4) {
      dq8<4>(grow[kk / 8], gs2, gb2, &ga);
      dq8<4>(urow[kk / 8], us2, ub2, &ua);
    } else {
      dq8_w8(grow[kk / 4], grow[kk / 4 + 1], gs2, gb2, &ga);
      dq8_w8(urow[kk / 4], urow[kk / 4 + 1], us2, ub2, &ua);
    }
    const f16x8 bvv = *reinterpret_cast<const f16x8*>(xrow + kk);
    gacc = __builtin_amdgcn_mfma_f32_16x16x32_f16(ga, bvv, gacc, 0, 0, 0);
    uacc = __builtin_amdgcn_mfma_f32_16x16x32_f16(ua, bvv, uacc, 0, 0, 0);
  }
#pragma unroll
  for (int r = 0; r < 4; ++r) {
    gacc[r] += gacc2[r];
    uacc[r] += uacc2[r];
  }

  const int tok = lane & 15;
  if (tok < cnt) {
#pragma unroll
    for (int reg = 0; reg < 4; ++reg) {
      const int o = row0 + (lane >> 4) * 4 + reg;
      if (o < I) {
        const float g = gacc[reg], u = uacc[reg];
        const float a = g / (1.0f + __expf(-g));
        h[(long)(p0 + tok) * I + o] = (_Float16)(a * u);
      }
    }
  }
}

template <int BITS, int GS>
__global__ __launch_bounds__(WF_BLOCK) void moe_w4f16_down_kernel(
    const _Float16* __restrict__ hh, const unsigned int* __restrict__ dq,
    const short* __restrict__ dsc, const short* __restrict__ dbi,
    float* __restrict__ out, const int* __restrict__ sub_expert,
    const int* __restrict__ sub_off, const int* __restrict__ sub_cnt,
    const int* __restrict__ sorted_tok, const float* __restrict__ sorted_wt,
    int I, int H) {
  const int s = blockIdx.y;
  const int e = sub_expert[s];
  const int p0 = sub_off[s];
  const int cnt = sub_cnt[s];
  if (cnt == 0) return;
  const int lane = threadIdx.x & (WAVE - 1);
  const int wid = threadIdx.x / WAVE;
  const int wpr = I * BITS / 32;

  const int row0 = (blockIdx.x * WF_WAVES + wid) * 16;
  if (row0 >= H) return;
  const int wr = min(row0 + (lane & 15), H - 1);
  const long ebase = (long)e * H;
  const unsigned int* drow = dq + (ebase + wr) * wpr;
  const int ngr = I / GS;
  const short* dsr = dsc + (ebase + wr) * ngr;
  const short* dbr = dbi + (ebase + wr) * ngr;
  const _Float16* hrow = hh + (long)(p0 + min(lane & 15, cnt - 1)) * I;

  float4v acc = {0, 0, 0, 0}, acc2 = {0, 0, 0, 0};
  constexpr float QOFF = BITS == 4 ? 8.0f : 128.0f;
  constexpr int WPS = BITS == 4 ? 1 : 2;

  const int nsl_total = I / 32;
  const int q = lane >> 4;
  int sl = 0;
  for (; sl + WF_NSL <= nsl_total; sl += WF_NSL) {
    uint4 dw4[2 * WPS];
    const int w0 = batch_kk(sl, q, 0) * BITS / 32;
#pragma unroll
    for (int c = 0; c < 2 * WPS; ++c)
      dw4[c] = *reinterpret_cast<const uint4*>(drow + w0 + c * 4);
    f16x8 bv[WF_NSL];
#pragma unroll
    for (int i = 0; i < WF_NSL; ++i)
      bv[i] = *reinterpret_cast<const f16x8*>(hrow + batch_kk(sl, q, i));
    LaneSB<GS> dsb;
    dsb.load(dsr, dbr, sl, q, QOFF);
    const unsigned int* dw = reinterpret_cast<const unsigned int*>(dw4);
    f16x8 da[WF_NSL];
#pragma unroll
    for (int i = 0; i < WF_NSL; ++i) {
      const int c = LaneSB<GS>::sel(i);
      if (BITS == 4)
        dq8<4>(dw[i], dsb.s2[c], dsb.b2[c], &da[i]);
      else
        dq8_w8(dw[i * 2], dw[i * 2 + 1], dsb.s2[c], dsb.b2[c], &da[i]);
    }
#pragma unroll
    for (int i = 0; i < WF_NSL; i += 2) {
      acc = __builtin_amdgcn_mfma_f32_16x16x32_f16(da[i], bv[i], acc, 0, 0, 0);
      acc2 = __builtin_amdgcn_mfma_f32_16x16x32_f16(da[i + 1], bv[i + 1],
                                                    acc2, 0, 0, 0);
    }
  }
  for (; sl < nsl_total; ++sl) {
    const int kk = sl * 32 + (lane >> 4) * 8;
    const float dsf = bfbits2f(dsr[kk / GS]);
    const f16x2 ds2 = splat2(dsf);
    const f16x2 db2 = splat2(bfbits2f(dbr[kk / GS]) + QOFF * dsf);
    f16x8 da;
    if (BITS == 4)
      dq8<4>(drow[kk / 8], ds2, db2, &da);
    else
      dq8_w8(drow[kk / 4], drow[kk / 4 + 1], ds2, db2, &da);
    const f16x8 bvv = *reinterpret_cast<const f16x8*>(hrow + kk);
    acc = __builtin_amdgcn_mfma_f32_16x16x32_f16(da, bvv, acc, 0, 0, 0);
  }
#pragma unroll
  for (int r = 0; r < 4; ++r) acc[r] += acc2[r];

  const int tok = lane & 15;
  if (tok < cnt) {
    const float wt = sorted_wt[p0 + tok];
    const long trow = (long)sorted_tok[p0 + tok] * H;
#pragma unroll
    for (int reg = 0; reg < 4; ++reg) {
      const int o = row0 + (lane >> 4) * 4 + reg;
      if (o < H) atomicAdd(out + trow + o, wt * acc[reg]);
    }
  }
}


#define NSL_D 4

__device__ __forceinline__ int batch_kk_d(int sl, int q, int i) {
  return sl * 32 + q * 32 + i * 8;
}

template <int GS>
struct LaneSBD {
  f16x2 s2, b2;
  __device__ __forceinline__ void load(const short* srow, const short* brow,
                                       int sl, int q, float qoff) {
    int g0;
    if (GS == 32) g0 = sl + q;
    else if (GS == 64) g0 = sl / 2 + (q >= 2 ? 1 : 0);
    else g0 = sl / 4;
    const float sf = bfbits2f(srow[g0]);
    s2 = splat2(sf);
    b2 = splat2(bfbits2f(brow[g0]) + qoff * sf);
  }
};

template <int MZ, int BITS, int GS>
__global__ __launch_bounds__(WF_BLOCK) void w4f16_gemv_kernel(
    const _Float16* __restrict__ x,
    const unsigned int* __restrict__ wq,
    const short* __restrict__ sc, const short* __restrict__ bi,
    short* __restrict__ y,
    float* __restrict__ yf,
    int M, int O, int H) {
  const int lane = threadIdx.x & (WAVE - 1);
  const int wid = threadIdx.x / WAVE;
  const int row0 = (blockIdx.x * WF_WAVES + wid) * 16;
  if (row0 >= O) return;
  const int wpr = H * BITS / 32;
  const int ngr = H / GS;
  const int wr = min(row0 + (lane & 15), O - 1);
  const unsigned int* wrow = wq + (long)wr * wpr;
  const short* srow = sc + (long)wr * ngr;
  const short* brow = bi + (long)wr * ngr;
  const _Float16* xrow[MZ];
#pragma unroll
  for (int z = 0; z < MZ; ++z)
    xrow[z] = x + (long)min(z * 16 + (lane & 15), M - 1) * H;

  float4v acc[MZ];
#pragma unroll
  for (int z = 0; z < MZ; ++z) acc[z] = float4v{0, 0, 0, 0};
  constexpr float QOFF = BITS == 4 ? 8.0f : 128.0f;
  constexpr int WPS = BITS == 4 ? 1 : 2;

  const int nsl_total = H / 32;
  const int nspb = ((nsl_total + gridDim.y - 1) / gridDim.y + NSL_D - 1) /
                   NSL_D * NSL_D;
  const int sl_lo = blockIdx.y * nspb;
  const int sl_hi = min(nsl_total, sl_lo + nspb);
  const int q = lane >> 4;

  int sl = sl_lo;
  for (; sl + NSL_D <= sl_hi; sl += NSL_D) {
    uint4 w4[WPS];
    const int w0 = batch_kk_d(sl, q, 0) * BITS / 32;
#pragma unroll
    for (int c = 0; c < WPS; ++c)
      w4[c] = *reinterpret_cast<const uint4*>(wrow + w0 + c * 4);
    f16x8 bv[MZ][NSL_D];
#pragma unroll
    for (int i = 0; i < NSL_D; ++i) {
      const int kk = batch_kk_d(sl, q, i);
#pragma unroll
      for (int z = 0; z < MZ; ++z)
        bv[z][i] = *reinterpret_cast<const f16x8*>(xrow[z] + kk);
    }
    LaneSBD<GS> sb;
    sb.load(srow, brow, sl, q, QOFF);
    const unsigned int* wbuf = reinterpret_cast<const unsigned int*>(w4);
#pragma unroll
    for (int i = 0; i < NSL_D; ++i) {
      f16x8 af;
      if (BITS == 4)
        dq8<4>(wbuf[i], sb.s2, sb.b2, &af);
      else
        dq8_w8(wbuf[i * 2], wbuf[i * 2 + 1], sb.s2, sb.b2, &af);
#pragma unroll
      for (int z = 0; z < MZ; ++z)
        acc[z] = __builtin_amdgcn_mfma_f32_16x16x32_f16(af, bv[z][i],
                                                        acc[z], 0, 0, 0);
    }
  }
  for (; sl < sl_hi; ++sl) {
    const int kk = sl * 32 + (lane >> 4) * 8;
    const float sf = bfbits2f(srow[kk / GS]);
    const f16x2 s2 = splat2(sf);
    const f16x2 b2 = splat2(bfbits2f(brow[kk / GS]) + QOFF * sf);
    f16x8 af;
    if (BITS == 4)
      dq8<4>(wrow[kk / 8], s2, b2, &af);
    else
      dq8_w8(wrow[kk / 4], wrow[kk / 4 + 1], s2, b2, &af);
#pragma unroll
    for (int z = 0; z < MZ; ++z) {
      const f16x8 bvv = *reinterpret_cast<const f16x8*>(xrow[z] + kk);
      acc[z] = __builtin_amdgcn_mfma_f32_16x16x32_f16(af, bvv, acc[z], 0, 0, 0);
    }
  }

#pragma unroll
  for (int z = 0; z < MZ; ++z)
    store_c_tile_lane(y, yf, acc[z], z * 16 + (lane & 15), M,
                      row0 + (lane >> 4) * 4, O);
}

extern "C" int w4f16_gemv_nsplit(int M, int O, int H) {
  const int gx = (O + WF_WAVES * 16 - 1) / (WF_WAVES * 16);
  const int nslt = H / 32;
  int nk = 256 / (gx > 0 ? gx : 1);
  const int max_nk = (nslt + NSL_D - 1) / NSL_D;
  if (nk > max_nk) nk = max_nk;
  if (nk < 1) nk = 1;
  return nk;
}

template <int BITS, int GS>
static void dispatch_gemv_mz(const void* x, const void* wq, const void* sc,
                             const void* bi, void* y, float* yf, int M,
                             int O, int H, int nk, hipStream_t stream) {
  const int gx = (O + WF_WAVES * 16 - 1) / (WF_WAVES * 16);
  const int mz = (M + 15) / 16;
  dim3 grid((unsigned)gx, (unsigned)nk);
  float* yfp = nk > 1 ? yf : nullptr;
#define GV_CASE(Z)                                                       \
  case Z:                                                                \
    w4f16_gemv_kernel<Z, BITS, GS><<<grid, dim3(WF_BLOCK), 0, stream>>>( \
        (const _Float16*)x, (const unsigned int*)wq, (const short*)sc,   \
        (const short*)bi, (short*)y, yfp, M, O, H);                      \
    break;
  switch (mz) {
    GV_CASE(1)
    GV_CASE(2)
    GV_CASE(3)
    GV_CASE(4)
    default:
      break;
  }
#undef GV_CASE
}

extern "C" void launch_w4f16_gemv(const void* x, const void* wq,
                                  const void* sc, const void* bi, void* y,
                                  float* yf, int nk, int M, int O, int H,
                                  int gs, int bits, hipStream_t stream) {
  if (nk > 1) launch_f32_zero(yf, (long)M * O, stream);
#define GV_GS(BB)                                                           \
  do {                                                                      \
    if (gs == 32)                                                           \
      dispatch_gemv_mz<BB, 32>(x, wq, sc, bi, y, yf, M, O, H, nk, stream);  \
    else if (gs == 64)                                                      \
      dispatch_gemv_mz<BB, 64>(x, wq, sc, bi, y, yf, M, O, H, nk, stream);  \
    else                                                                    \
      dispatch_gemv_mz<BB, 128>(x, wq, sc, bi, y, yf, M, O, H, nk, stream); \
  } while (0)
  if (bits == 4) GV_GS(4);
  else GV_GS(8);
#undef GV_GS
  if (nk > 1) launch_f32_to_bf16(yf, y, (long)M * O, stream);
}

template <int BITS>
static void dispatch_gateup(const void* x, const void* gq, const void* uq,
                            const void* gsc, const void* gbi, const void* usc,
                            const void* ubi, void* h, const int* se,
                            const int* so, const int* sc, const int* st,
                            int S, int H, int I, int gs, hipStream_t stream) {
  const int gx = (I + WF_WAVES * 16 - 1) / (WF_WAVES * 16);
  dim3 grid(gx, S), block(WF_BLOCK);
#define GU_CASE(GSV)                                                        \
  moe_w4f16_gateup_kernel<BITS, GSV><<<grid, block, 0, stream>>>(           \
      (const _Float16*)x, (const unsigned int*)gq, (const unsigned int*)uq, \
      (const short*)gsc, (const short*)gbi, (const short*)usc,              \
      (const short*)ubi, (_Float16*)h, se, so, sc, st, H, I)
  if (gs == 32) GU_CASE(32);
  else if (gs == 64) GU_CASE(64);
  else GU_CASE(128);
#undef GU_CASE
}

extern "C" void launch_moe_w4f16_gateup(
    const void* x, const void* gq, const void* uq, const void* gsc,
    const void* gbi, const void* usc, const void* ubi, void* h,
    const int* sub_expert, const int* sub_off, const int* sub_cnt,
    const int* sorted_tok, int S, int H, int I, int gs, int bits,
    hipStream_t stream) {
  if (bits == 4)
    dispatch_gateup<4>(x, gq, uq, gsc, gbi, usc, ubi, h, sub_expert, sub_off,
                       sub_cnt, sorted_tok, S, H, I, gs, stream);
  else
    dispatch_gateup<8>(x, gq, uq, gsc, gbi, usc, ubi, h, sub_expert, sub_off,
                       sub_cnt, sorted_tok, S, H, I, gs, stream);
}

template <int BITS>
static void dispatch_down(const void* hh, const void* dq, const void* dsc,
                          const void* dbi, float* out, const int* se,
                          const int* so, const int* sc, const int* st,
                          const float* sw, int S, int I, int H, int gs,
                          hipStream_t stream) {
  const int gx = (H + WF_WAVES * 16 - 1) / (WF_WAVES * 16);
  dim3 grid(gx, S), block(WF_BLOCK);
#define DN_CASE(GSV)                                                      \
  moe_w4f16_down_kernel<BITS, GSV><<<grid, block, 0, stream>>>(           \
      (const _Float16*)hh, (const unsigned int*)dq, (const short*)dsc,    \
      (const short*)dbi, out, se, so, sc, st, sw, I, H)
  if (gs == 32) DN_CASE(32);
  else if (gs == 64) DN_CASE(64);
  else DN_CASE(128);
#undef DN_CASE
}

extern "C" void launch_moe_w4f16_down(
    const void* hh, const void* dq, const void* dsc, const void* dbi,
    float* out, const int* sub_expert, const int* sub_off, const int* sub_cnt,
    const int* sorted_tok, const float* sorted_wt, int S, int I, int H,
    int gs, int bits, hipStream_t stream) {
  if (bits == 4)
    dispatch_down<4>(hh, dq, dsc, dbi, out, sub_expert, sub_off, sub_cnt,
                     sorted_tok, sorted_wt, S, I, H, gs, stream);
  else
    dispatch_down<8>(hh, dq, dsc, dbi, out, sub_expert, sub_off, sub_cnt,
                     sorted_tok, sorted_wt, S, I, H, gs, stream);
}
```

### mlx_sharding_amd/ops/kvcache.py

```python

from __future__ import annotations

from typing import List, Optional, Tuple

import torch


class KVCache:
    CHUNK = 1024

    def __init__(self, n_kv_heads: int, k_head_dim: int, v_head_dim: int,
                 dtype: torch.dtype = torch.bfloat16,
                 device: torch.device | str = "cpu",
                 batch_size: int = 1):
        self.n_kv_heads = n_kv_heads
        self.k_head_dim = k_head_dim
        self.v_head_dim = v_head_dim
        if not dtype.is_floating_point:
            raise TypeError(f"KV cache dtype must be floating, got {dtype}")
        self.dtype = dtype
        self.device = torch.device(device)
        self.batch_size = batch_size
        self.offset = 0
        self._k: Optional[torch.Tensor] = None
        self._v: Optional[torch.Tensor] = None
        self.graph_pos: Optional[torch.Tensor] = None
        self._fixed = False

    def _ensure(self, batch: int, needed: int):
        cap = 0 if self._k is None else self._k.shape[2]
        if self._k is not None and self._k.shape[0] != batch:
            raise ValueError(f"KV cache batch mismatch: {self._k.shape[0]} vs {batch}")
        if needed <= cap and self._k is not None:
            return
        if self._fixed:
            raise ValueError(f"KV cache capacity {cap} is fixed; "
                             f"{needed} positions needed")
        new_cap = ((needed + self.CHUNK - 1) // self.CHUNK) * self.CHUNK
        nk = torch.empty(batch, self.n_kv_heads, new_cap, self.k_head_dim,
                         dtype=self.dtype, device=self.device)
        nv = torch.empty(batch, self.n_kv_heads, new_cap, self.v_head_dim,
                         dtype=self.dtype, device=self.device)
        if self._k is not None and self.offset > 0:
            nk[:, :, : self.offset] = self._k[:, :, : self.offset]
            nv[:, :, : self.offset] = self._v[:, :, : self.offset]
        self._k, self._v = nk, nv

    def update(self, k: torch.Tensor, v: torch.Tensor) -> Tuple[torch.Tensor, torch.Tensor]:
        if self.graph_pos is not None:
            idx = self.graph_pos.to(torch.long)
            if idx.numel() > 1:
                rows = torch.arange(idx.numel(), device=idx.device)
                self._k[rows, :, idx] = k[:, :, 0]
                self._v[rows, :, idx] = v[:, :, 0]
                return self._k, self._v
            self._k.index_copy_(2, idx, k)
            self._v.index_copy_(2, idx, v)
            return self._k, self._v
        B, H, T, _ = k.shape
        self._ensure(B, self.offset + T)
        self._k[:, :, self.offset: self.offset + T] = k
        self._v[:, :, self.offset: self.offset + T] = v
        self.offset += T
        return (self._k[:, :, : self.offset], self._v[:, :, : self.offset])

    def append_mla(self, kvh: torch.Tensor, kpe: torch.Tensor):
        from .. import ops as _ops
        ext = _ops.hip_ext()
        B, T = kvh.shape[0], kvh.shape[1]
        if self.graph_pos is not None:
            ext.mla_append_kv(kvh, kpe, self._k, self._v,
                              pos=self.graph_pos)
            return self._k, self._v
        self._ensure(B, self.offset + T)
        ext.mla_append_kv(kvh, kpe, self._k, self._v, pos0=self.offset)
        self.offset += T
        return (self._k[:, :, : self.offset], self._v[:, :, : self.offset])

    def append_rope_kv(self, k: torch.Tensor, v: torch.Tensor,
                       cos: torch.Tensor, sin: torch.Tensor,
                       interleaved: bool = False):
        from .. import ops as _ops
        ext = _ops.hip_ext()
        B, T = k.shape[0], k.shape[1]
        if self.graph_pos is not None:
            ext.rope_append_kv(k, v, cos, sin, self._k, self._v,
                               pos=self.graph_pos, interleaved=interleaved)
            return self._k, self._v
        self._ensure(B, self.offset + T)
        ext.rope_append_kv(k, v, cos, sin, self._k, self._v,
                           pos0=self.offset, interleaved=interleaved)
        self.offset += T
        return (self._k[:, :, : self.offset], self._v[:, :, : self.offset])

    @property
    def k(self) -> Optional[torch.Tensor]:
        return None if self._k is None else self._k[:, :, : self.offset]

    @property
    def v(self) -> Optional[torch.Tensor]:
        return None if self._v is None else self._v[:, :, : self.offset]

    def keys_buffer(self) -> Optional[torch.Tensor]:
        return self._k

    def values_buffer(self) -> Optional[torch.Tensor]:
        return self._v

    @property
    def capacity(self) -> int:
        return 0 if self._k is None else self._k.shape[2]

    def ensure_capacity(self, cap: int, batch: Optional[int] = None):
        b = batch if batch is not None else (
            self._k.shape[0] if self._k is not None else self.batch_size)
        self._ensure(b, cap)

    def allocate(self, capacity: int, batch: Optional[int] = None):
        b = batch if batch is not None else self.batch_size
        shape = (b, self.n_kv_heads, capacity)
        self._k = torch.zeros(*shape, self.k_head_dim, dtype=self.dtype,
                              device=self.device)
        self._v = torch.zeros(*shape, self.v_head_dim, dtype=self.dtype,
                              device=self.device)
        self.batch_size = b
        self._fixed = True

    def slot(self, i: int) -> "KVCache":
        if self._k is None or not 0 <= i < self._k.shape[0]:
            raise IndexError(f"slot {i} outside the allocated pool")
        c = KVCache(self.n_kv_heads, self.k_head_dim, self.v_head_dim,
                    dtype=self.dtype, device=self.device, batch_size=1)
        c._k, c._v = self._k[i:i + 1], self._v[i:i + 1]
        c._fixed = True
        return c

    def trim(self, n: int):
        if n < 0 or n > self.offset:
            raise ValueError(f"trim({n}) outside [0, {self.offset}]")
        self.offset = n
        self.graph_pos = None

    def reset(self):
        self.offset = 0
        self.graph_pos = None


def make_cache(layer_specs: List[Tuple[int, int, int]], dtype: torch.dtype,
               device, batch_size: int = 1) -> List[KVCache]:
    return [KVCache(h, kd, vd, dtype=dtype, device=device, batch_size=batch_size)
            for (h, kd, vd) in layer_specs]
```

Before: 6615 tokens/s.

## Fuse MLA decode prep and MoE finalize into dedicated decode kernels

Adds a decode-only path for DeepSeek-V2 MLA attention: one kernel applies the kv layernorm, writes RoPE'd keys into the cache and prepares q_pe/q_nope. Attention then runs on the absorbed latent cache via strided attn_decode_split instead of materialising per-head K/V. For MoE decode it emits an f16 copy of the normed input from rms_norm_residual, clears the fp32 accumulator inside the gate/up kernel, and fuses the shared-expert add and residual add into a single finalize kernel. The aim is fewer small kernel launches and less intermediate memory traffic per decode step, at the cost of more specialised code paths and a different bf16 rounding order.

Result: faster. 7564 tokens/s, median of 6 (+14.3%).

```diff
diff --git a/mlx_sharding_amd/models/deepseek_v2.py b/mlx_sharding_amd/models/deepseek_v2.py
--- a/mlx_sharding_amd/models/deepseek_v2.py
+++ b/mlx_sharding_amd/models/deepseek_v2.py
@@ -36,24 +36,25 @@
             self.quant.group_size, self.quant.bits)
 
     def forward_subs(self, x_flat: torch.Tensor, subs,
-                     max_tok: int = 4) -> torch.Tensor:
+                     max_tok: int = 4, raw: bool = False) -> torch.Tensor:
         if self.quant is not None:
             import os
             if os.environ.get("MLXS_AMD_MOE_RESIDENT"):
                 dense = self.resident_dense()
                 if dense is not None:
                     return ops.grouped_expert_mlp_subs(
-                        x_flat, dense[0], dense[1], dense[2], subs, max_tok)
+                        x_flat, dense[0], dense[1], dense[2], subs, max_tok,
+                        raw=raw)
             g, u, d = self.gate_proj, self.up_proj, self.down_proj
             return ops.grouped_expert_mlp_quant_subs(
                 x_flat,
                 (g.weight, g.scales, g.biases),
                 (u.weight, u.scales, u.biases),
                 (d.weight, d.scales, d.biases),
-                subs, self.quant.group_size, self.quant.bits)
+                subs, self.quant.group_size, self.quant.bits, raw=raw)
         return ops.grouped_expert_mlp_subs(
             x_flat, self.gate_proj.weight, self.up_proj.weight,
-            self.down_proj.weight, subs, max_tok)
+            self.down_proj.weight, subs, max_tok, raw=raw)
 
     def forward(self, x_flat: torch.Tensor, weights: torch.Tensor,
                 indices: torch.Tensor) -> torch.Tensor:
@@ -179,6 +180,11 @@
         else:
             qh = self.q_proj(x)
         qh = qh.view(B, T, nh, self.qk_head_dim)
+        if (T == 1 and ops.use_native(x) and ops.decode_fuse_enabled()
+                and self.qk_nope % 8 == 0 and rope % 2 == 0):
+            if ckv is None:
+                ckv = self.kv_a_proj_with_mqa(x)
+            return self._decode_fused(qh, ckv, cos, sin, cache)
         q_nope = qh[..., : self.qk_nope]
         q_pe = ops.apply_rope(qh[..., self.qk_nope:], cos, sin,
                               interleaved=True)
@@ -230,6 +236,23 @@
         qf = torch.cat([q_nope, q_pe], dim=-1).transpose(1, 2)
         out = ops.attention(qf, k, v, self.scale, causal_offset=offset)
         return self.o_proj(out.transpose(1, 2).reshape(B, T, -1))
+
+    def _decode_fused(self, qh, ckv, cos, sin, cache: KVCache):
+        B = qh.shape[0]
+        nh, rank = self.n_heads, self.kv_lora_rank
+        gp = cache.graph_pos
+        ln = self.kv_a_layernorm
+        q_pe, qn, k_all = cache.mla_decode_prep(
+            qh, ckv, ln.weight, ln.eps, ln.weight_offset, cos, sin,
+            self.qk_rope)
+        self._ensure_absorb(qh.device, qh.dtype)
+        q_abs = torch.bmm(qn, self._w_uk)
+        o = ops.hip_ext().attn_decode_split(
+            q_abs.transpose(0, 1), q_pe, k_all, k_all[..., :rank],
+            self.scale, 0.0, 0, gp)
+        ov = torch.bmm(o, self._w_uv)
+        out = ov.view(nh, B, 1, self.v_head_dim).permute(1, 2, 0, 3)
+        return self.o_proj(out.reshape(B, 1, -1))
 
     def _forward_naive(self, x, cos, sin, cache: Optional[KVCache]):
         B, T, _ = x.shape
@@ -317,9 +340,31 @@
                 and 1 <= topk_group <= n_group
                 and topk_group * (E // n_group) >= K)
 
-    def forward(self, x):
+    def packed_decode(self, n_tokens: int) -> bool:
+        import os
+        return (self.switch_mlp.quant is not None
+                and not os.environ.get("MLXS_AMD_MOE_RESIDENT")
+                and self._fused_gate_ok(n_tokens))
+
+    def forward(self, x, residual=None):
         B, T, H = x.shape
         flat = x.reshape(-1, H)
+        if (residual is not None and ops.use_native(flat)
+                and self._fused_gate_ok(flat.shape[0])):
+            f16 = getattr(x, "_mlxs_f16", None)
+            if f16 is not None:
+                flat._mlxs_f16 = f16.view(-1, H)
+            logits = self.gate(flat.to(self.gate.weight.dtype))
+            n_group, topk_group = self._gate_groups()
+            subs = ops.moe_gate_subranges(logits, self.top_k,
+                                          self.routed_scaling_factor,
+                                          self.norm_topk_prob, max_tok=16,
+                                          n_group=n_group,
+                                          topk_group=topk_group)
+            acc = self.switch_mlp.forward_subs(flat, subs, 16, raw=True)
+            shared = (self.shared_experts(flat)
+                      if self.shared_experts is not None else None)
+            return ops.moe_finalize(acc, shared, residual)
         if (ops.use_native(flat)
                 and self._fused_gate_ok(flat.shape[0])):
             logits = self.gate(flat.to(self.gate.weight.dtype))
@@ -362,6 +407,14 @@
     def forward(self, x, cos, sin, cache):
         attn = self.self_attn(self.input_layernorm(x), cos, sin, cache)
         pn = self.post_attention_layernorm
+        if (x.shape[1] == 1 and ops.use_native(x)
+                and ops.decode_fuse_enabled()
+                and isinstance(self.mlp, DeepseekV2MoE)
+                and self.mlp._fused_gate_ok(x.shape[0])):
+            y, h = ops.rms_norm_residual(
+                attn, x, pn.weight, pn.eps, pn.weight_offset,
+                want_f16=self.mlp.packed_decode(x.shape[0]))
+            return self.mlp(y, residual=h)
         y, h = ops.rms_norm_residual(attn, x, pn.weight, pn.eps,
                                      pn.weight_offset)
         return h + self.mlp(y)
diff --git a/mlx_sharding_amd/ops/__init__.py b/mlx_sharding_amd/ops/__init__.py
--- a/mlx_sharding_amd/ops/__init__.py
+++ b/mlx_sharding_amd/ops/__init__.py
@@ -63,10 +63,20 @@
     return ref.rms_norm(x, weight, eps, weight_offset)
 
 
-def rms_norm_residual(x, residual, weight, eps: float = 1e-5, weight_offset: float = 0.0):
-    if _use_hip(x):
-        y, h = _require_ext("rms_norm_residual").rms_norm_residual(
-            x, residual, weight, eps, weight_offset)
+def decode_fuse_enabled() -> bool:
+    return not os.environ.get("MLXS_AMD_NO_DECODE_FUSE")
+
+
+def rms_norm_residual(x, residual, weight, eps: float = 1e-5,
+                      weight_offset: float = 0.0, want_f16: bool = False):
+    if _use_hip(x):
+        ext = _require_ext("rms_norm_residual")
+        if want_f16:
+            y, h, y16 = ext.rms_norm_residual(x, residual, weight, eps,
+                                              weight_offset, True)
+            y._mlxs_f16 = y16
+            return y, h
+        y, h = ext.rms_norm_residual(x, residual, weight, eps, weight_offset)
         return y, h
     h = x + residual
     return ref.rms_norm(h, weight, eps, weight_offset), h
@@ -354,7 +364,14 @@
                                         norm_topk_prob, n_group, topk_group))
 
 
-def grouped_expert_mlp_subs(x, gate_w, up_w, down_w, subs, max_tok: int = 4):
+def moe_finalize(acc, shared, h):
+    return _require_ext("moe_finalize").moe_finalize(
+        acc, None if shared is None else shared.reshape(acc.shape),
+        h.reshape(acc.shape)).view(h.shape)
+
+
+def grouped_expert_mlp_subs(x, gate_w, up_w, down_w, subs, max_tok: int = 4,
+                            raw: bool = False):
     ext = _require_ext("grouped_expert_mlp")
     sub_e, sub_off, sub_cnt, sorted_tok, sorted_wt = subs
     P = sorted_tok.shape[0]
@@ -362,7 +379,7 @@
                                sorted_tok, P, max_tok)
     out = ext.moe_down_grouped(h, down_w, sub_e, sub_off, sub_cnt,
                                sorted_tok, sorted_wt, x.shape[0], max_tok)
-    return out.to(x.dtype)
+    return out if raw else out.to(x.dtype)
 
 
 def _to_f16_cached(x: torch.Tensor) -> torch.Tensor:
@@ -401,7 +418,8 @@
 
 
 def grouped_expert_mlp_quant_subs(x, gate, up, down, subs,
-                                  group_size: int, bits: int):
+                                  group_size: int, bits: int,
+                                  raw: bool = False):
     ext = _require_ext("grouped_expert_mlp_quant")
     sub_e, sub_off, sub_cnt, sorted_tok, sorted_wt = subs
     P = sorted_tok.shape[0]
@@ -413,6 +431,14 @@
     gq = repack_w4(gate[0], bits)
     uq = repack_w4(up[0], bits)
     dq = repack_w4(down[0], bits)
+    if raw:
+        hh, acc = ext.moe_w4f16_gateup_acc(
+            x16, gq, uq, gate[1], gate[2], up[1], up[2], sub_e, sub_off,
+            sub_cnt, sorted_tok, P, group_size, bits, x.shape[0],
+            down[0].shape[1])
+        return ext.moe_w4f16_down(hh, dq, down[1], down[2], sub_e, sub_off,
+                                  sub_cnt, sorted_tok, sorted_wt, x.shape[0],
+                                  group_size, bits, acc)
     hh = ext.moe_w4f16_gateup(x16, gq, uq, gate[1], gate[2], up[1], up[2],
                               sub_e, sub_off, sub_cnt, sorted_tok, P,
                               group_size, bits)
diff --git a/mlx_sharding_amd/ops/hip/attn_decode.hip b/mlx_sharding_amd/ops/hip/attn_decode.hip
--- a/mlx_sharding_amd/ops/hip/attn_decode.hip
+++ b/mlx_sharding_amd/ops/hip/attn_decode.hip
@@ -6,6 +6,7 @@
 template <int G, int DVT>
 __global__ __launch_bounds__(AD_BLOCK) void attn_decode_kernel(
     const short* __restrict__ q,
+    const short* __restrict__ q_rope,
     const short* __restrict__ kcache,
     const short* __restrict__ vcache,
     short* __restrict__ out,
@@ -14,7 +15,8 @@
     const int* __restrict__ s_ptr,
     int s_bstride,
     int B, int Hq, int Hkv, int S, long Scap, int Dk, int Dv, long vstride,
-    float scale, float softcap, int window) {
+    float scale, float softcap, int window, int Dr, long q_bs, long q_hs,
+    long qr_bs, long qr_hs, long o_bs, long o_hs) {
   const int b = blockIdx.x / Hkv;
   if (s_ptr) S = s_ptr[b * s_bstride] + 1;
   const int hk = blockIdx.x % Hkv;
@@ -31,9 +33,11 @@
       smem_raw + (((size_t)G * Dk * sizeof(short) + 15) & ~(size_t)15));
   float* red = p_lds + (size_t)G * AD_BLOCK;
 
+  const int Dn = Dk - Dr;
   for (int i = tid; i < G * Dk; i += AD_BLOCK) {
     int g = i / Dk, d = i % Dk;
-    q_lds[i] = q[((long)b * Hq + h0 + g) * Dk + d];
+    q_lds[i] = d < Dn ? q[b * q_bs + (h0 + g) * q_hs + d]
+                      : q_rope[b * qr_bs + (h0 + g) * qr_hs + d - Dn];
   }
   __syncthreads();
 
@@ -194,7 +198,7 @@
       for (int u = 0; u < DVT; ++u) {
         const int dv = tid + u * AD_BLOCK;
         if (dv < Dv)
-          ((bf16*)out)[((long)b * Hq + h0 + g) * Dv + dv] =
+          ((bf16*)out)[b * o_bs + (h0 + g) * o_hs + dv] =
               f2bf(acc[g * DVT + u] / l[g]);
       }
     return;
@@ -223,8 +227,9 @@
     const float* __restrict__ part_o,
     const float* __restrict__ part_ml,
     short* __restrict__ out,
-    int NS, int Dv) {
+    int NS, int Dv, int Hq, long o_bs, long o_hs) {
   const long bh = blockIdx.x;
+  short* orow = out + (bh / Hq) * o_bs + (bh % Hq) * o_hs;
   const int tid = threadIdx.x;
   float mstar = -1e30f;
   for (int s = 0; s < NS; ++s)
@@ -241,17 +246,20 @@
       const float ms = part_ml[(bh * NS + s) * 2];
       o += part_o[(bh * NS + s) * Dv + d] * __expf(ms - mstar);
     }
-    ((bf16*)out)[bh * Dv + d] = f2bf(o / lsum);
+    ((bf16*)orow)[d] = f2bf(o / lsum);
   }
 }
 
-extern "C" void launch_attn_decode(const void* q, const void* k, const void* v,
+extern "C" void launch_attn_decode(const void* q, const void* q_rope,
+                                   const void* k, const void* v,
                                    void* out, float* part_o, float* part_ml,
                                    int nsplit, const int* s_ptr,
                                    int s_bstride, int B, int Hq,
                                    int Hkv, int S, long Scap, int Dk, int Dv,
                                    long vstride, float scale, float softcap,
-                                   int window, hipStream_t stream) {
+                                   int window, int Dr, long q_bs, long q_hs,
+                                   long qr_bs, long qr_hs, long o_bs,
+                                   long o_hs, hipStream_t stream) {
   const int Gtot = Hq / Hkv;
   const int DVT = (Dv + AD_BLOCK - 1) / AD_BLOCK;
   const int G = (Gtot == 16 && DVT == 2) ? 8 : Gtot;
@@ -264,9 +272,10 @@
 #define AD_CASE(GG, VT)                                                      \
   case GG * 16 + VT:                                                         \
     attn_decode_kernel<GG, VT><<<grid, block, smem, stream>>>(               \
-        (const short*)q, (const short*)k, (const short*)v, (short*)out,      \
-        part_o, part_ml, s_ptr, s_bstride, B, Hq, Hkv, S, Scap, Dk, Dv,      \
-        vstride, scale, softcap, window);                                    \
+        (const short*)q, (const short*)q_rope, (const short*)k,              \
+        (const short*)v, (short*)out, part_o, part_ml, s_ptr, s_bstride, B,  \
+        Hq, Hkv, S, Scap, Dk, Dv, vstride, scale, softcap, window, Dr, q_bs, \
+        q_hs, qr_bs, qr_hs, o_bs, o_hs);                                     \
     break;
   switch (G * 16 + DVT) {
     AD_CASE(1, 1)
@@ -286,7 +295,7 @@
   if (nsplit > 1) {
     attn_decode_combine_kernel<<<dim3((unsigned)(B * Hq)), dim3(128), 0,
                                  stream>>>(part_o, part_ml, (short*)out,
-                                           nsplit, Dv);
+                                           nsplit, Dv, Hq, o_bs, o_hs);
   }
 }
 
diff --git a/mlx_sharding_amd/ops/hip/bindings.hip b/mlx_sharding_amd/ops/hip/bindings.hip
--- a/mlx_sharding_amd/ops/hip/bindings.hip
+++ b/mlx_sharding_amd/ops/hip/bindings.hip
@@ -8,8 +8,15 @@
 void launch_rms_norm(const void*, void*, const void*, long, int, float, float,
                      long, hipStream_t);
 void launch_rms_norm_residual(const void*, const void*, void*, void*,
-                              const void*, long, int, float, float,
+                              const void*, long, int, float, float, void*,
                               hipStream_t);
+void launch_mla_decode_prep(const void*, const void*, const void*,
+                            const float*, const float*, void*, void*, void*,
+                            const int*, int, int, int, int, int, int, int,
+                            long, long, long, long, long, float, float,
+                            hipStream_t);
+void launch_moe_finalize(const float*, const void*, const void*, void*, long,
+                         hipStream_t);
 void launch_glu(const void*, const void*, void*, long, bool, hipStream_t);
 void launch_glu_strided(const void*, const void*, void*, long, int, long,
                         long, bool, hipStream_t);
@@ -23,9 +30,10 @@
                            const float*, void*, void*, const int*, int, int,
                            int, int, int, int, long, bool, long, long, long,
                            hipStream_t);
-void launch_attn_decode(const void*, const void*, const void*, void*, float*,
-                        float*, int, const int*, int, int, int, int, int,
-                        long, int, int, long, float, float, int, hipStream_t);
+void launch_attn_decode(const void*, const void*, const void*, const void*,
+                        void*, float*, float*, int, const int*, int, int, int,
+                        int, int, long, int, int, long, float, float, int,
+                        int, long, long, long, long, long, long, hipStream_t);
 bool attn_decode_supported_shape(int, int);
 void launch_attn_prefill(const void*, const void*, const void*, void*, int,
                          int, int, int, int, long, long, int, int, float,
@@ -72,7 +80,7 @@
                              const void*, const void*, const void*,
                              const void*, void*, const int*, const int*,
                              const int*, const int*, int, int, int, int, int,
-                             hipStream_t);
+                             float*, long, hipStream_t);
 void launch_moe_w4f16_down(const void*, const void*, const void*, const void*,
                            float*, const int*, const int*, const int*,
                            const int*, const float*, int, int, int, int, int,
@@ -177,7 +185,7 @@
 std::vector<torch::Tensor> rms_norm_residual(torch::Tensor x,
                                              torch::Tensor resid,
                                              torch::Tensor w, double eps,
-                                             double w_off) {
+                                             double w_off, bool with_f16) {
   check_bf16(x, "x");
   auto xc = x.contiguous();
   auto rc = resid.contiguous();
@@ -185,10 +193,87 @@
   long rows = xc.numel() / H;
   auto y = torch::empty_like(xc);
   auto h = torch::empty_like(xc);
+  torch::Tensor y16;
+  if (with_f16) y16 = torch::empty_like(xc, xc.options().dtype(torch::kHalf));
   launch_rms_norm_residual(xc.data_ptr(), rc.data_ptr(), y.data_ptr(),
                            h.data_ptr(), w.contiguous().data_ptr(), rows, H,
-                           (float)eps, (float)w_off, cur_stream());
+                           (float)eps, (float)w_off,
+                           with_f16 ? y16.data_ptr() : nullptr, cur_stream());
+  if (with_f16) return {y, h, y16};
   return {y, h};
+}
+
+std::vector<torch::Tensor> mla_decode_prep(
+    torch::Tensor qh, torch::Tensor ckv, torch::Tensor w, double eps,
+    double w_off, torch::Tensor cos, torch::Tensor sin, torch::Tensor cache,
+    int64_t rope, c10::optional<torch::Tensor> pos, int64_t pos0) {
+  check_bf16(qh, "qh");
+  check_bf16(ckv, "ckv");
+  check_bf16(w, "w");
+  check_bf16(cache, "cache");
+  TORCH_CHECK(qh.dim() == 4 && qh.size(1) == 1, "qh must be [B, 1, nh, D]");
+  TORCH_CHECK(ckv.dim() == 3 && ckv.size(1) == 1 && ckv.size(0) == qh.size(0),
+              "ckv must be [B, 1, rank+rope]");
+  const int B = qh.size(0), nh = qh.size(2);
+  const int nope = qh.size(3) - rope;
+  const int rank = ckv.size(2) - rope;
+  TORCH_CHECK(rope >= 2 && rope % 2 == 0 && nope >= 8 && nope % 8 == 0 &&
+                  rank >= 4 && rank % 4 == 0,
+              "mla_decode_prep needs rope % 2 == 0, nope % 8 == 0, "
+              "rank % 4 == 0 (got rope=", rope, ", nope=", nope, ", rank=",
+              rank, ")");
+  TORCH_CHECK(w.numel() == rank, "norm weight must hold rank elements");
+  TORCH_CHECK(cache.dim() == 4 && cache.is_contiguous() &&
+                  cache.size(0) == B && cache.size(1) == 1 &&
+                  cache.size(3) == rank + rope,
+              "cache must be contiguous [B, 1, Scap, rank+rope]");
+  const long Scap = cache.size(2);
+  auto cc = cos.contiguous();
+  auto sc = sin.contiguous();
+  const long csb = rope_table_bstride(cc, sc, B, 1, rope / 2);
+  int pbs;
+  const int* pp = pos_arg(pos, B, pbs);
+  if (!pp)
+    TORCH_CHECK(pos0 >= 0 && pos0 < Scap, "position ", pos0,
+                " outside the cache capacity ", Scap);
+  torch::Tensor qv = qh, cv = ckv;
+  if (!(qh.stride(3) == 1 && qh.stride(1) % 8 == 0 && qh.stride(2) % 8 == 0 &&
+        (B == 1 || qh.stride(0) % 8 == 0) &&
+        ((uintptr_t)qh.data_ptr()) % 16 == 0))
+    qv = qh.contiguous();
+  if (!(ckv.stride(2) == 1 && (B == 1 || ckv.stride(0) % 4 == 0) &&
+        ((uintptr_t)ckv.data_ptr()) % 8 == 0))
+    cv = ckv.contiguous();
+  auto q_pe = torch::empty({B, nh, rope}, qh.options());
+  auto q_nope = torch::empty({nh, B, nope}, qh.options());
+  launch_mla_decode_prep(qv.data_ptr(), cv.data_ptr(),
+                         w.contiguous().data_ptr(), cc.data_ptr<float>(),
+                         sc.data_ptr<float>(), cache.data_ptr(),
+                         q_pe.data_ptr(), q_nope.data_ptr(), pp, pbs,
+                         (int)pos0, B, nh, nope, (int)rope, rank, Scap,
+                         qv.stride(0), qv.stride(2), cv.stride(0), csb,
+                         (float)eps, (float)w_off, cur_stream());
+  return {q_pe, q_nope};
+}
+
+torch::Tensor moe_finalize(torch::Tensor acc, c10::optional<torch::Tensor> shared,
+                           torch::Tensor h) {
+  check_bf16(h, "h");
+  TORCH_CHECK(acc.is_cuda() && acc.scalar_type() == torch::kFloat32 &&
+                  acc.is_contiguous(), "acc must be contiguous fp32 on GPU");
+  TORCH_CHECK(h.numel() == acc.numel(), "h/acc size mismatch");
+  auto hc = h.contiguous();
+  torch::Tensor sc;
+  if (shared.has_value()) {
+    check_bf16(*shared, "shared");
+    TORCH_CHECK(shared->numel() == acc.numel(), "shared/acc size mismatch");
+    sc = shared->contiguous();
+  }
+  auto out = torch::empty(h.sizes(), hc.options());
+  launch_moe_finalize(acc.data_ptr<float>(),
+                      sc.defined() ? sc.data_ptr() : nullptr, hc.data_ptr(),
+                      out.data_ptr(), acc.numel(), cur_stream());
+  return out;
 }
 
 torch::Tensor glu(torch::Tensor gate, torch::Tensor up, bool gelu) {
@@ -308,14 +393,15 @@
                        cur_stream());
 }
 
-torch::Tensor attn_decode(torch::Tensor q, torch::Tensor k, torch::Tensor v,
-                          double scale, double softcap, int64_t window,
-                          c10::optional<torch::Tensor> pos) {
-  check_bf16(q, "q");
+torch::Tensor attn_decode_impl(const torch::Tensor& qn, const torch::Tensor& qr,
+                               torch::Tensor k, torch::Tensor v, double scale,
+                               double softcap, int64_t window,
+                               c10::optional<torch::Tensor> pos,
+                               bool head_major) {
   check_bf16(k, "k");
-  TORCH_CHECK(q.size(2) == 1, "attn_decode needs Tq == 1");
-  auto qc = q.contiguous();
-  const int B = qc.size(0), Hq = qc.size(1), Dk = qc.size(3);
+  const torch::Tensor& qc = qn;
+  const int Dr = qr.defined() ? (int)qr.size(2) : 0;
+  const int B = qn.size(0), Hq = qn.size(1), Dk = qn.size(2) + Dr;
   const int Hkv = k.size(1), S = k.size(2);
   const int Dv = v.size(3);
   TORCH_CHECK(k.stride(3) == 1 && v.stride(3) == 1, "K/V rows must be contiguous");
@@ -330,7 +416,10 @@
   long kScap = k.stride(1) / Dk;
   long vScap = v.stride(1) / vstride;
   TORCH_CHECK(kScap == vScap, "K/V capacity mismatch");
-  auto out = torch::empty({B, Hq, 1, Dv}, qc.options());
+  auto out = head_major ? torch::empty({Hq, B, Dv}, qc.options())
+                        : torch::empty({B, Hq, 1, Dv}, qc.options());
+  const long o_bs = head_major ? Dv : (long)Hq * Dv;
+  const long o_hs = head_major ? (long)B * Dv : Dv;
   int sbs;
   const int* s_ptr = pos_arg(pos, B, sbs);
   long span = s_ptr ? kScap : (long)S;
@@ -348,11 +437,40 @@
     part_o = po.data_ptr<float>();
     part_ml = pml.data_ptr<float>();
   }
-  launch_attn_decode(qc.data_ptr(), k.data_ptr(), v.data_ptr(),
-                     out.data_ptr(), part_o, part_ml, nsplit, s_ptr, sbs, B,
-                     Hq, Hkv, S, kScap, Dk, Dv, vstride, (float)scale,
-                     (float)softcap, (int)window, cur_stream());
+  launch_attn_decode(qn.data_ptr(), Dr ? qr.data_ptr() : nullptr,
+                     k.data_ptr(), v.data_ptr(), out.data_ptr(), part_o,
+                     part_ml, nsplit, s_ptr, sbs, B, Hq, Hkv, S, kScap, Dk,
+                     Dv, vstride, (float)scale, (float)softcap, (int)window,
+                     Dr, qn.stride(0), qn.stride(1), Dr ? qr.stride(0) : 0,
+                     Dr ? qr.stride(1) : 0, o_bs, o_hs, cur_stream());
   return out;
+}
+
+torch::Tensor attn_decode(torch::Tensor q, torch::Tensor k, torch::Tensor v,
+                          double scale, double softcap, int64_t window,
+                          c10::optional<torch::Tensor> pos) {
+  check_bf16(q, "q");
+  TORCH_CHECK(q.dim() == 4 && q.size(2) == 1, "attn_decode needs Tq == 1");
+  auto qc = q.contiguous();
+  return attn_decode_impl(qc.view({qc.size(0), qc.size(1), qc.size(3)}),
+                          torch::Tensor(), k, v, scale, softcap, window, pos,
+                          false);
+}
+
+torch::Tensor attn_decode_split(torch::Tensor q_nope, torch::Tensor q_rope,
+                                torch::Tensor k, torch::Tensor v, double scale,
+                                double softcap, int64_t window,
+                                c10::optional<torch::Tensor> pos) {
+  check_bf16(q_nope, "q_nope");
+  check_bf16(q_rope, "q_rope");
+  TORCH_CHECK(q_nope.dim() == 3 && q_rope.dim() == 3 &&
+                  q_nope.size(0) == q_rope.size(0) &&
+                  q_nope.size(1) == q_rope.size(1) && q_rope.size(2) > 0,
+              "q_nope/q_rope must be [B, Hq, *] with matching B, Hq");
+  TORCH_CHECK(q_nope.stride(2) == 1 && q_rope.stride(2) == 1,
+              "q rows must be contiguous");
+  return attn_decode_impl(q_nope, q_rope, k, v, scale, softcap, window, pos,
+                          true);
 }
 
 torch::Tensor attn_prefill(torch::Tensor q, torch::Tensor k, torch::Tensor v,
@@ -574,13 +692,14 @@
   return y;
 }
 
-torch::Tensor moe_w4f16_gateup(torch::Tensor x, torch::Tensor gq,
-                               torch::Tensor uq, torch::Tensor gsc,
-                               torch::Tensor gbi, torch::Tensor usc,
-                               torch::Tensor ubi, torch::Tensor sub_expert,
-                               torch::Tensor sub_off, torch::Tensor sub_cnt,
-                               torch::Tensor sorted_tok, int64_t P,
-                               int64_t gs, int64_t bits) {
+torch::Tensor moe_w4f16_gateup_impl(torch::Tensor x, torch::Tensor gq,
+                                    torch::Tensor uq, torch::Tensor gsc,
+                                    torch::Tensor gbi, torch::Tensor usc,
+                                    torch::Tensor ubi, torch::Tensor sub_expert,
+                                    torch::Tensor sub_off, torch::Tensor sub_cnt,
+                                    torch::Tensor sorted_tok, int64_t P,
+                                    int64_t gs, int64_t bits,
+                                    const torch::Tensor& clear) {
   TORCH_CHECK(x.scalar_type() == torch::kHalf, "x must be fp16");
   const int H = x.size(1);
   const int I = gq.size(1);
@@ -593,8 +712,35 @@
       gbi.data_ptr(), usc.data_ptr(), ubi.data_ptr(), h.data_ptr(),
       sub_expert.data_ptr<int>(), sub_off.data_ptr<int>(),
       sub_cnt.data_ptr<int>(), sorted_tok.data_ptr<int>(), S, H, I, (int)gs,
-      (int)bits, cur_stream());
+      (int)bits, clear.defined() ? clear.data_ptr<float>() : nullptr,
+      clear.defined() ? clear.numel() : 0, cur_stream());
   return h;
+}
+
+torch::Tensor moe_w4f16_gateup(torch::Tensor x, torch::Tensor gq,
+                               torch::Tensor uq, torch::Tensor gsc,
+                               torch::Tensor gbi, torch::Tensor usc,
+                               torch::Tensor ubi, torch::Tensor sub_expert,
+                               torch::Tensor sub_off, torch::Tensor sub_cnt,
+                               torch::Tensor sorted_tok, int64_t P,
+                               int64_t gs, int64_t bits) {
+  return moe_w4f16_gateup_impl(x, gq, uq, gsc, gbi, usc, ubi, sub_expert,
+                               sub_off, sub_cnt, sorted_tok, P, gs, bits,
+                               torch::Tensor());
+}
+
+std::vector<torch::Tensor> moe_w4f16_gateup_acc(
+    torch::Tensor x, torch::Tensor gq, torch::Tensor uq, torch::Tensor gsc,
+    torch::Tensor gbi, torch::Tensor usc, torch::Tensor ubi,
+    torch::Tensor sub_expert, torch::Tensor sub_off, torch::Tensor sub_cnt,
+    torch::Tensor sorted_tok, int64_t P, int64_t gs, int64_t bits, int64_t N,
+    int64_t Hout) {
+  TORCH_CHECK(N >= 1 && Hout >= 1, "accumulator shape must be positive");
+  auto acc = torch::empty({N, Hout}, x.options().dtype(torch::kFloat32));
+  auto h = moe_w4f16_gateup_impl(x, gq, uq, gsc, gbi, usc, ubi, sub_expert,
+                                 sub_off, sub_cnt, sorted_tok, P, gs, bits,
+                                 acc);
+  return {h, acc};
 }
 
 torch::Tensor moe_w4f16_down(torch::Tensor hh, torch::Tensor dq,
@@ -602,14 +748,23 @@
                              torch::Tensor sub_expert, torch::Tensor sub_off,
                              torch::Tensor sub_cnt, torch::Tensor sorted_tok,
                              torch::Tensor sorted_wt, int64_t N, int64_t gs,
-                             int64_t bits) {
+                             int64_t bits, c10::optional<torch::Tensor> acc) {
   TORCH_CHECK(hh.scalar_type() == torch::kHalf, "h must be fp16");
   const int I = hh.size(1);
   const int H = dq.size(1);
   const int S = sub_expert.size(0);
   TORCH_CHECK(I % 32 == 0, "I%32 required");
   TORCH_CHECK(gs == 32 || gs == 64 || gs == 128, "gs must be 32/64/128");
-  auto out = torch::zeros({N, H}, hh.options().dtype(torch::kFloat32));
+  torch::Tensor out;
+  if (acc.has_value()) {
+    out = *acc;
+    TORCH_CHECK(out.is_cuda() && out.scalar_type() == torch::kFloat32 &&
+                    out.is_contiguous() && out.dim() == 2 &&
+                    out.size(0) == N && out.size(1) == H,
+                "acc must be contiguous fp32 [N, H]");
+  } else {
+    out = torch::zeros({N, H}, hh.options().dtype(torch::kFloat32));
+  }
   launch_moe_w4f16_down(
       hh.contiguous().data_ptr(), dq.data_ptr(), dsc.data_ptr(),
       dbi.data_ptr(), out.data_ptr<float>(), sub_expert.data_ptr<int>(),
@@ -684,7 +839,16 @@
 
 PYBIND11_MODULE(TORCH_EXTENSION_NAME, m) {
   m.def("rms_norm", &rms_norm, "fused RMSNorm (gfx950)");
-  m.def("rms_norm_residual", &rms_norm_residual);
+  m.def("rms_norm_residual", &rms_norm_residual, pybind11::arg("x"),
+        pybind11::arg("resid"), pybind11::arg("w"), pybind11::arg("eps"),
+        pybind11::arg("w_off"), pybind11::arg("with_f16") = false);
+  m.def("mla_decode_prep", &mla_decode_prep, pybind11::arg("qh"),
+        pybind11::arg("ckv"), pybind11::arg("w"), pybind11::arg("eps"),
+        pybind11::arg("w_off"), pybind11::arg("cos"), pybind11::arg("sin"),
+        pybind11::arg("cache"), pybind11::arg("rope"),
+        pybind11::arg("pos") = pybind11::none(), pybind11::arg("pos0") = 0);
+  m.def("moe_finalize", &moe_finalize, pybind11::arg("acc"),
+        pybind11::arg("shared"), pybind11::arg("h"));
   m.def("glu", &glu);
   m.def("softcap", &softcap_op);
   m.def("apply_rope", &apply_rope);
@@ -699,6 +863,10 @@
         pybind11::arg("pos0") = 0);
   m.def("attn_decode", &attn_decode, pybind11::arg("q"), pybind11::arg("k"),
         pybind11::arg("v"), pybind11::arg("scale"), pybind11::arg("softcap"),
+        pybind11::arg("window"), pybind11::arg("pos") = pybind11::none());
+  m.def("attn_decode_split", &attn_decode_split, pybind11::arg("q_nope"),
+        pybind11::arg("q_rope"), pybind11::arg("k"), pybind11::arg("v"),
+        pybind11::arg("scale"), pybind11::arg("softcap"),
         pybind11::arg("window"), pybind11::arg("pos") = pybind11::none());
   m.def("attn_decode_shape_ok", [](int64_t g, int64_t dv) {
     return attn_decode_supported_shape((int)g, (int)dv);
@@ -725,7 +893,13 @@
   m.def("moe_down_grouped", &moe_down_grouped);
   m.def("moe_w4_mfma", &moe_w4_mfma);
   m.def("moe_w4f16_gateup", &moe_w4f16_gateup);
-  m.def("moe_w4f16_down", &moe_w4f16_down);
+  m.def("moe_w4f16_gateup_acc", &moe_w4f16_gateup_acc);
+  m.def("moe_w4f16_down", &moe_w4f16_down, pybind11::arg("hh"),
+        pybind11::arg("dq"), pybind11::arg("dsc"), pybind11::arg("dbi"),
+        pybind11::arg("sub_expert"), pybind11::arg("sub_off"),
+        pybind11::arg("sub_cnt"), pybind11::arg("sorted_tok"),
+        pybind11::arg("sorted_wt"), pybind11::arg("N"), pybind11::arg("gs"),
+        pybind11::arg("bits"), pybind11::arg("acc") = pybind11::none());
   m.def("moe_gate_subranges", &moe_gate_subranges, pybind11::arg("logits"),
         pybind11::arg("top_k"), pybind11::arg("s_upper"),
         pybind11::arg("max_tok"), pybind11::arg("routed_scaling"),
diff --git a/mlx_sharding_amd/ops/hip/elementwise.hip b/mlx_sharding_amd/ops/hip/elementwise.hip
--- a/mlx_sharding_amd/ops/hip/elementwise.hip
+++ b/mlx_sharding_amd/ops/hip/elementwise.hip
@@ -1,5 +1,7 @@
 #include "hip_common.h"
 
+
+typedef _Float16 f16x4v __attribute__((ext_vector_type(4)));
 
 template <int BLOCK, bool RESIDUAL>
 __global__ void rms_norm_kernel(const short* __restrict__ x,
@@ -7,7 +9,8 @@
                                 short* __restrict__ y,
                                 short* __restrict__ h_out,
                                 const short* __restrict__ w, int H, float eps,
-                                float w_off, long xstride) {
+                                float w_off, long xstride,
+                                _Float16* __restrict__ y16) {
   __shared__ float scratch[BLOCK / WAVE];
   const long row = blockIdx.x;
   const short* xr = x + row * xstride;
@@ -53,6 +56,11 @@
     o.z = (short)__bfloat16_as_ushort(f2bf(bfbits2f(v.z) * inv * (bfbits2f(wvv.z) + w_off)));
     o.w = (short)__bfloat16_as_ushort(f2bf(bfbits2f(v.w) * inv * (bfbits2f(wvv.w) + w_off)));
     reinterpret_cast<short4v*>(yr)[i] = o;
+    if (y16) {
+      f16x4v o16 = {(_Float16)bfbits2f(o.x), (_Float16)bfbits2f(o.y),
+                    (_Float16)bfbits2f(o.z), (_Float16)bfbits2f(o.w)};
+      reinterpret_cast<f16x4v*>(y16 + row * H)[i] = o16;
+    }
   }
 }
 
@@ -62,17 +70,18 @@
   constexpr int BLOCK = 256;
   rms_norm_kernel<BLOCK, false><<<dim3((unsigned)rows), dim3(BLOCK), 0, stream>>>(
       (const short*)x, nullptr, (short*)y, nullptr, (const short*)w, H, eps,
-      w_off, xstride);
+      w_off, xstride, nullptr);
 }
 
 extern "C" void launch_rms_norm_residual(const void* x, const void* resid,
                                          void* y, void* h_out, const void* w,
                                          long rows, int H, float eps,
-                                         float w_off, hipStream_t stream) {
+                                         float w_off, void* y16,
+                                         hipStream_t stream) {
   constexpr int BLOCK = 256;
   rms_norm_kernel<BLOCK, true><<<dim3((unsigned)rows), dim3(BLOCK), 0, stream>>>(
       (const short*)x, (const short*)resid, (short*)y, (short*)h_out,
-      (const short*)w, H, eps, w_off, H);
+      (const short*)w, H, eps, w_off, H, (_Float16*)y16);
 }
 
 
@@ -344,3 +353,154 @@
                                    rope, Scap,
                                    kpe_rstride);
 }
+
+
+#define PREP_BLOCK 256
+
+__device__ __forceinline__ void rope_pair_pinned(float x1, float x2, float c,
+                                                 float s, float& o1,
+                                                 float& o2) {
+#pragma clang fp contract(off)
+  const float x2s = x2 * s;
+  const float x1s = x1 * s;
+  o1 = __builtin_fmaf(x1, c, -x2s);
+  o2 = __builtin_fmaf(x2, c, x1s);
+}
+
+__global__ __launch_bounds__(PREP_BLOCK) void mla_decode_prep_kernel(
+    const short* __restrict__ qh, const short* __restrict__ ckv,
+    const short* __restrict__ w, const float* __restrict__ cost,
+    const float* __restrict__ sint, short* __restrict__ cache,
+    short* __restrict__ q_pe_out, short* __restrict__ q_nope_out,
+    const int* __restrict__ pos_ptr, int pos_bstride, int pos0, int B, int nh,
+    int nope, int rope, int rank, long Scap, long q_rs, long q_hs, long ckv_rs,
+    long cs_bstride, float eps, float w_off, int n_pe_blocks) {
+  __shared__ float scratch[PREP_BLOCK / WAVE];
+  const int b = blockIdx.x;
+  const int half = rope / 2;
+  const float* c = cost + (long)b * cs_bstride;
+  const float* s = sint + (long)b * cs_bstride;
+
+  if (blockIdx.y == 0) {
+    const long pos = pos_ptr ? pos_ptr[b * pos_bstride] : pos0;
+    const short* xr = ckv + (long)b * ckv_rs;
+    float ss = 0.0f;
+    const int nvec = rank / 4;
+    const short4v* xv = reinterpret_cast<const short4v*>(xr);
+    for (int i = threadIdx.x; i < nvec; i += PREP_BLOCK) {
+      short4v v = xv[i];
+      float f0 = bfbits2f(v.x), f1 = bfbits2f(v.y), f2 = bfbits2f(v.z),
+            f3 = bfbits2f(v.w);
+      {
+#pragma clang fp contract(off)
+        ss += f0 * f0 + f1 * f1 + f2 * f2 + f3 * f3;
+      }
+    }
+    ss = block_sum<PREP_BLOCK>(ss, scratch);
+    if (pos < 0 || pos >= Scap) return;
+    const float inv = rsqrtf(ss / (float)rank + eps);
+    short* krow = cache + ((long)b * Scap + pos) * (rank + rope);
+    const short4v* wv = reinterpret_cast<const short4v*>(w);
+    for (int i = threadIdx.x; i < nvec; i += PREP_BLOCK) {
+      short4v v = xv[i];
+      short4v wvv = wv[i];
+      short4v o;
+      o.x = (short)__bfloat16_as_ushort(f2bf(bfbits2f(v.x) * inv * (bfbits2f(wvv.x) + w_off)));
+      o.y = (short)__bfloat16_as_ushort(f2bf(bfbits2f(v.y) * inv * (bfbits2f(wvv.y) + w_off)));
+      o.z = (short)__bfloat16_as_ushort(f2bf(bfbits2f(v.z) * inv * (bfbits2f(wvv.z) + w_off)));
+      o.w = (short)__bfloat16_as_ushort(f2bf(bfbits2f(v.w) * inv * (bfbits2f(wvv.w) + w_off)));
+      reinterpret_cast<short4v*>(krow)[i] = o;
+    }
+    const short* pe = xr + rank;
+    for (int p = threadIdx.x; p < half; p += PREP_BLOCK) {
+      const float x1 = bfbits2f(pe[2 * p]), x2 = bfbits2f(pe[2 * p + 1]);
+      float o1, o2;
+      rope_pair_pinned(x1, x2, c[p], s[p], o1, o2);
+      krow[rank + 2 * p] = (short)__bfloat16_as_ushort(f2bf(o1));
+      krow[rank + 2 * p + 1] = (short)__bfloat16_as_ushort(f2bf(o2));
+    }
+    return;
+  }
+
+  const short* qrow = qh + (long)b * q_rs;
+  if ((int)blockIdx.y <= n_pe_blocks) {
+    const int idx = (blockIdx.y - 1) * PREP_BLOCK + threadIdx.x;
+    if (idx >= nh * half) return;
+    const int head = idx / half, p = idx - head * half;
+    const short* xr = qrow + (long)head * q_hs + nope;
+    short* yr = q_pe_out + ((long)b * nh + head) * rope;
+    const float x1 = bfbits2f(xr[2 * p]), x2 = bfbits2f(xr[2 * p + 1]);
+    float o1, o2;
+    rope_pair_pinned(x1, x2, c[p], s[p], o1, o2);
+    yr[2 * p] = (short)__bfloat16_as_ushort(f2bf(o1));
+    yr[2 * p + 1] = (short)__bfloat16_as_ushort(f2bf(o2));
+    return;
+  }
+
+  const int nv8 = nope / 8;
+  const int idx = (blockIdx.y - 1 - n_pe_blocks) * PREP_BLOCK + threadIdx.x;
+  if (idx >= nh * nv8) return;
+  const int head = idx / nv8, v = idx - head * nv8;
+  reinterpret_cast<short8v*>(q_nope_out + ((long)head * B + b) * nope)[v] =
+      *reinterpret_cast<const short8v*>(qrow + (long)head * q_hs + v * 8);
+}
+
+extern "C" void launch_mla_decode_prep(
+    const void* qh, const void* ckv, const void* w, const float* cost,
+    const float* sint, void* cache, void* q_pe_out, void* q_nope_out,
+    const int* pos_ptr, int pos_bstride, int pos0, int B, int nh, int nope,
+    int rope, int rank, long Scap, long q_rs, long q_hs, long ckv_rs,
+    long cs_bstride, float eps, float w_off, hipStream_t stream) {
+  const int n_pe = (nh * (rope / 2) + PREP_BLOCK - 1) / PREP_BLOCK;
+  const int n_cp = (nh * (nope / 8) + PREP_BLOCK - 1) / PREP_BLOCK;
+  mla_decode_prep_kernel<<<dim3((unsigned)B, (unsigned)(1 + n_pe + n_cp)),
+                           dim3(PREP_BLOCK), 0, stream>>>(
+      (const short*)qh, (const short*)ckv, (const short*)w, cost, sint,
+      (short*)cache, (short*)q_pe_out, (short*)q_nope_out, pos_ptr,
+      pos_bstride, pos0, B, nh, nope, rope, rank, Scap, q_rs, q_hs, ckv_rs,
+      cs_bstride, eps, w_off, n_pe);
+}
+
+
+__device__ __forceinline__ short bf_round_bits(float v) {
+  return (short)__bfloat16_as_ushort(f2bf(v));
+}
+
+__global__ void moe_finalize_kernel(const float* __restrict__ acc,
+                                    const short* __restrict__ shared,
+                                    const short* __restrict__ h,
+                                    short* __restrict__ out, long n) {
+  const long stride = (long)gridDim.x * blockDim.x;
+  const long n4 = n / 4;
+  for (long i = blockIdx.x * blockDim.x + threadIdx.x; i < n4; i += stride) {
+    const float4v a = reinterpret_cast<const float4v*>(acc)[i];
+    const short4v hv = reinterpret_cast<const short4v*>(h)[i];
+    short4v sv = {0, 0, 0, 0};
+    if (shared) sv = reinterpret_cast<const short4v*>(shared)[i];
+    short4v o;
+#pragma unroll
+    for (int k = 0; k < 4; ++k) {
+      short y = bf_round_bits(a[k]);
+      if (shared) y = bf_round_bits(bfbits2f(y) + bfbits2f(sv[k]));
+      o[k] = bf_round_bits(bfbits2f(hv[k]) + bfbits2f(y));
+    }
+    reinterpret_cast<short4v*>(out)[i] = o;
+  }
+  for (long i = n4 * 4 + blockIdx.x * blockDim.x + threadIdx.x; i < n;
+       i += stride) {
+    short y = bf_round_bits(acc[i]);
+    if (shared) y = bf_round_bits(bfbits2f(y) + bfbits2f(shared[i]));
+    out[i] = bf_round_bits(bfbits2f(h[i]) + bfbits2f(y));
+  }
+}
+
+extern "C" void launch_moe_finalize(const float* acc, const void* shared,
+                                    const void* h, void* out, long n,
+                                    hipStream_t stream) {
+  const int block = 256;
+  long want = (n / 4 + block - 1) / block;
+  int grid = (int)min(want, (long)(256 * 8));
+  if (grid < 1) grid = 1;
+  moe_finalize_kernel<<<dim3(grid), dim3(block), 0, stream>>>(
+      acc, (const short*)shared, (const short*)h, (short*)out, n);
+}
diff --git a/mlx_sharding_amd/ops/hip/moe_w4f16.hip b/mlx_sharding_amd/ops/hip/moe_w4f16.hip
--- a/mlx_sharding_amd/ops/hip/moe_w4f16.hip
+++ b/mlx_sharding_amd/ops/hip/moe_w4f16.hip
@@ -42,7 +42,16 @@
     const short* __restrict__ ubi, _Float16* __restrict__ h,
     const int* __restrict__ sub_expert, const int* __restrict__ sub_off,
     const int* __restrict__ sub_cnt, const int* __restrict__ sorted_tok,
-    int H, int I) {
+    int H, int I, float* __restrict__ clear, long clear_n) {
+  if (clear) {
+    const long nthr = (long)gridDim.x * gridDim.y * WF_BLOCK;
+    const long t0 =
+        ((long)blockIdx.y * gridDim.x + blockIdx.x) * WF_BLOCK + threadIdx.x;
+    const long n4 = clear_n / 4;
+    for (long i = t0; i < n4; i += nthr)
+      reinterpret_cast<float4v*>(clear)[i] = float4v{0, 0, 0, 0};
+    for (long i = n4 * 4 + t0; i < clear_n; i += nthr) clear[i] = 0.0f;
+  }
   const int s = blockIdx.y;
   const int e = sub_expert[s];
   const int p0 = sub_off[s];
@@ -416,14 +425,15 @@
                             const void* gsc, const void* gbi, const void* usc,
                             const void* ubi, void* h, const int* se,
                             const int* so, const int* sc, const int* st,
-                            int S, int H, int I, int gs, hipStream_t stream) {
+                            int S, int H, int I, int gs, float* clear,
+                            long clear_n, hipStream_t stream) {
   const int gx = (I + WF_WAVES * 16 - 1) / (WF_WAVES * 16);
   dim3 grid(gx, S), block(WF_BLOCK);
 #define GU_CASE(GSV)                                                        \
   moe_w4f16_gateup_kernel<BITS, GSV><<<grid, block, 0, stream>>>(           \
       (const _Float16*)x, (const unsigned int*)gq, (const unsigned int*)uq, \
       (const short*)gsc, (const short*)gbi, (const short*)usc,              \
-      (const short*)ubi, (_Float16*)h, se, so, sc, st, H, I)
+      (const short*)ubi, (_Float16*)h, se, so, sc, st, H, I, clear, clear_n)
   if (gs == 32) GU_CASE(32);
   else if (gs == 64) GU_CASE(64);
   else GU_CASE(128);
@@ -435,13 +445,15 @@
     const void* gbi, const void* usc, const void* ubi, void* h,
     const int* sub_expert, const int* sub_off, const int* sub_cnt,
     const int* sorted_tok, int S, int H, int I, int gs, int bits,
-    hipStream_t stream) {
+    float* clear, long clear_n, hipStream_t stream) {
   if (bits == 4)
     dispatch_gateup<4>(x, gq, uq, gsc, gbi, usc, ubi, h, sub_expert, sub_off,
-                       sub_cnt, sorted_tok, S, H, I, gs, stream);
+                       sub_cnt, sorted_tok, S, H, I, gs, clear, clear_n,
+                       stream);
   else
     dispatch_gateup<8>(x, gq, uq, gsc, gbi, usc, ubi, h, sub_expert, sub_off,
-                       sub_cnt, sorted_tok, S, H, I, gs, stream);
+                       sub_cnt, sorted_tok, S, H, I, gs, clear, clear_n,
+                       stream);
 }
 
 template <int BITS>
diff --git a/mlx_sharding_amd/ops/kvcache.py b/mlx_sharding_amd/ops/kvcache.py
--- a/mlx_sharding_amd/ops/kvcache.py
+++ b/mlx_sharding_amd/ops/kvcache.py
@@ -77,6 +77,22 @@
         self.offset += T
         return (self._k[:, :, : self.offset], self._v[:, :, : self.offset])
 
+    def mla_decode_prep(self, qh: torch.Tensor, ckv: torch.Tensor, norm_w,
+                        eps: float, w_off: float, cos, sin, rope: int):
+        from .. import ops as _ops
+        ext = _ops.hip_ext()
+        B = qh.shape[0]
+        if self.graph_pos is not None:
+            q_pe, qn = ext.mla_decode_prep(qh, ckv, norm_w, eps, w_off, cos,
+                                           sin, self._k, rope,
+                                           pos=self.graph_pos)
+            return q_pe, qn, self._k
+        self._ensure(B, self.offset + 1)
+        q_pe, qn = ext.mla_decode_prep(qh, ckv, norm_w, eps, w_off, cos, sin,
+                                       self._k, rope, pos0=self.offset)
+        self.offset += 1
+        return q_pe, qn, self._k[:, :, : self.offset]
+
     def append_rope_kv(self, k: torch.Tensor, v: torch.Tensor,
                        cos: torch.Tensor, sin: torch.Tensor,
                        interleaved: bool = False):
```
